# Draghoyns/FLAIR-1

Hardware: AMD Instinct MI355X
Metric: 512x512x5 tiles/s (train fwd+bwd) (higher is better)
Workload: dtype bf16; 1 GPU; U-Net/ResNet34 5-ch 512x512 13-class train step (fwd + fused CE/argmax/confmat + bwd + SGD), bs=32/GPU, random-init weights; global_batch=32, parallelism=dp1, grad_allreduce=none

## Files before the change

flair-1_amd/build.py:

```python
#!/usr/bin/env python3
import os
import subprocess
import sys
from concurrent.futures import ThreadPoolExecutor

HERE = os.path.dirname(os.path.abspath(__file__))
CSRC = os.path.join(HERE, "csrc")
OUT_DIR = os.path.join(HERE, "flair_amd")
OBJ_DIR = os.path.join(HERE, "build")
LIB = os.path.join(OUT_DIR, "libflair_hip.so")
SOURCES = ["conv_igemm.hip", "conv_halo.hip", "conv_hg.hip", "wgrad.hip", "wgrad_halo.hip", "wgrad_hg.hip", "stem.hip", "batchnorm.hip", "misc.hip", "ce_head.hip", "feed.hip", "zone_stitch.hip", "zone_metrics.hip", "tiff_lzw.hip", "tiff_read.hip", "unet.hip", "capi.hip", "prof.hip", "tune.hip", "metadata_mlp.hip", "tf_exec.hip", "segformer_ops.hip", "segformer.hip", "swin_ops.hip", "upernet.hip"]
FLAGS = ["--offload-arch=gfx950", "-O3", "-std=c++17", "-fPIC", "-Wall", "-Wno-unused-function"]
SOURCE_FLAGS = {src: ["-fno-slp-vectorize"] for src in ("feed.hip", "zone_stitch.hip", "zone_metrics.hip")}
if os.environ.get("FLAIR_STAMPS") == "1":
    FLAGS.append("-DFLAIR_HG_STAMPS")


def _hipcc():
    for c in (os.environ.get("HIPCC"), "/opt/rocm/bin/hipcc", "hipcc"):
        if c and (os.path.isabs(c) and os.path.exists(c) or not os.path.isabs(c)):
            return c
    return "hipcc"


def _newer(target, deps):
    if not os.path.exists(target):
        return False
    t = os.path.getmtime(target)
    return all(os.path.getmtime(d) <= t for d in deps)


def build(force=False, verbose=True):
    os.makedirs(OBJ_DIR, exist_ok=True)
    headers = [os.path.join(CSRC, f) for f in os.listdir(CSRC) if f.endswith(".h")]
    headers.append(os.path.join(os.path.dirname(HERE), "include", "flair_hip.h"))
    hipcc = _hipcc()
    jobs = []
    objs = []
    for src in SOURCES:
        s = os.path.join(CSRC, src)
        o = os.path.join(OBJ_DIR, src.replace(".hip", ".o"))
        objs.append(o)
        if force or not _newer(o, [s] + headers):
            jobs.append([hipcc] + FLAGS + SOURCE_FLAGS.get(src, []) + ["-c", s, "-o", o])

    def run(cmd):
        if verbose:
            print(" ".join(cmd), flush=True)
        r = subprocess.run(cmd, capture_output=True, text=True)
        if r.returncode != 0:
            raise RuntimeError("hipcc failed:\n" + " ".join(cmd) + "\n" + r.stdout + r.stderr)
        if verbose and r.stderr.strip():
            print(r.stderr, flush=True)

    with ThreadPoolExecutor(max_workers=4) as ex:
        list(ex.map(run, jobs))
    if force or jobs or not os.path.exists(LIB):
        run([hipcc, "--offload-arch=gfx950", "-shared", "-fPIC", "-o", LIB] + objs)
    return LIB


if __name__ == "__main__":
    print(build(force="--force" in sys.argv))
```

flair-1_amd/csrc/capi.hip:

```cpp
#include <new>
#include <string.h>

#include "../../include/flair_hip.h"
#include "unet.h"
#include "conv_args.h"
#include "parity_pack.h"
#include "segformer.h"
#include "upernet.h"
#include "segformer_ops.h"
#include "swin_ops.h"

using namespace flair;

struct flair_unet { UNet net; flair_unet(int a, int b, int c) : net(a, b, c) {} };
struct flair_segformer {
  SegFormer net;
  flair_segformer(int a, int b, const int* d, const int* h, const int* hd, const int* sr, int dh, int dt) : net(a, b, d, h, hd, sr, dh, dt) {}
};

struct flair_upernet {
  UperNet net;
  flair_upernet(int a, int b, int e, const int* d, const int* h, int hid, const int* ps, int ai, int ac, int dt)
      : net(a, b, e, d, h, hid, ps, ai, ac, dt) {}
};
// ... 468 lines not shown
  ConvArgs a;
  float standin;
  if (!p || conv_ex_fill(p, a)) return 0;
  conv_ex_sizing(p, a, &standin);
  if (p->mode == 2) {
    PackTable tb;
    return conv_ex_parity_packs(p, a, nullptr, tb) + 256;
  }
  a.stats = p->stats;
  size_t b = (size_t)round_up((long)((size_t)conv_weight_rows_pad(p->Cout) * a.Kpad * dtype_size(p->dtype)), 256);
  if (p->stats) b += (size_t)round_up((long)conv_grid_rows(p->dtype, a) * 2 * p->Cout * 4, 256);
  return b + 256;
}

int flair_conv2d_ex_grid_rows(const flair_conv_ex_t* p) {
  ConvArgs a;
  float standin;
  if (!p) return -1;
  const int rc = conv_ex_fill(p, a);
  if (rc) return rc;
  conv_ex_sizing(p, a, &standin);
  a.stats = p->stats;
  return conv_grid_rows(p->dtype, a);
}

int flair_conv2d_ex(const flair_conv_ex_t* p, void* workspace, size_t wsb, void* stream) {
  if (!p || !p->x0 || !p->w_oihw || !workspace) return -1;
  hipStream_t s = (hipStream_t)stream;
  ConvArgs a;
  int rc = conv_ex_fill(p, a);
  if (rc) return rc;
  if (p->mode == 2) {
    if (!p->y_nhwc) return -1;
    PackTable tb;
    if (conv_ex_parity_packs(p, a, (unsigned char*)workspace, tb) > wsb) return -100;
    rc = pack_weights_all(p->dtype, p->w_oihw, workspace, tb, s);
    return rc ? rc : launch_conv(p->dtype, a, s);
  }
  if (p->bnr_partial ? (!p->bnr_y || !p->bnr_scale || !p->bnr_shift) : (p->bnr_y != nullptr)) return -1;
  OpArena ar(workspace, wsb);
  const int Cin = a.C0 + a.C1, rows_f = conv_weight_rows_pad(p->Cout);
  void* wp = ar.get((size_t)rows_f * a.Kpad * dtype_size(p->dtype));
  a.w = wp;
  if (p->bnr_partial && p->bnr_rows < conv_grid_rows(p->dtype, a)) return -100;
  float* partial = nullptr;
  int nblk = 0;
  if (p->stats) {
    a.stats = p->stats;
    nblk = conv_grid_rows(p->dtype, a);
    partial = (float*)ar.get((size_t)nblk * 2 * p->Cout * 4);
    a.stats = partial;
  }
  if (ar.bad) return -100;
  rc = p->mode == 1 ? pack_weight(p->dtype, p->w_oihw, wp, Cin, p->Cout, p->R, p->R, Cin, rows_f, a.Kpad, 1, s)
                    : pack_weight(p->dtype, p->w_oihw, wp, p->Cout, Cin, p->R, p->R, Cin, rows_f, a.Kpad, 0, s);
  if (rc) return rc;
  rc = launch_conv(p->dtype, a, s);
  if (rc) return rc;
  if (p->stats) rc = partial_rows_sum(partial, nblk, 2 * p->Cout, p->stats, s);
  return rc;
}

static int wgrad_ex_fill(const flair_wgrad_ex_t* p, WgradArgs& w) {
  if (p->dtype != DT_F32 && p->dtype != DT_BF16) return -2;
  const ConvInput in{p->x0, p->x1, p->C0, p->x1 ? p->C1 : 0, p->up0, p->N, p->H, p->W};
  wgrad_args(w, in, p->R, p->stride, p->pad, p->dy, p->dy_ld > 0 ? p->dy_ld : p->Cout, p->Cout, p->dw,
             p->Cin_real > 0 ? p->Cin_real : in.C0 + in.C1);
  w.accumulate = p->accumulate; w.in_scale = p->in_scale; w.in_shift = p->in_shift; w.cus = p->cus; w.dbias = p->dbias;
  w.fuse_y = p->fuse_y; w.fuse_coef = p->fuse_coef; w.fuse_msc = p->fuse_msc; w.fuse_msh = p->fuse_msh;
  return 0;
}

size_t flair_conv2d_wgrad_ex_workspace_bytes(const flair_wgrad_ex_t* p) {
  WgradArgs w;
  if (!p || wgrad_ex_fill(p, w)) return 0;
  size_t b = (size_t)round_up((long)wgrad_workspace_bytes(p->dtype, w), 256);
  if (p->dbias && wgrad_dbias_fusable(p->dtype, w)) b += (size_t)round_up((long)WGRAD_DBIAS_ROWS * w.dy_ld * 4, 256);
  return b + 256;
}

int flair_conv2d_wgrad_ex(const flair_wgrad_ex_t* p, void* workspace, size_t wsb, void* stream) {
  if (!p || !p->x0 || !p->dy || !p->dw || !workspace) return -1;
  WgradArgs w;
  int rc = wgrad_ex_fill(p, w);
  if (rc) return rc;
  OpArena ar(workspace, wsb);
  w.partial = (float*)ar.get(wgrad_workspace_bytes(p->dtype, w));
  if (p->dbias && wgrad_dbias_fusable(p->dtype, w)) w.dbias_partial = (float*)ar.get((size_t)WGRAD_DBIAS_ROWS * w.dy_ld * 4);
  if (ar.bad) return -100;
  return launch_wgrad(p->dtype, w, (hipStream_t)stream);
}

size_t flair_bn_workspace_bytes(int64_t rows, int C) {
  if (rows < 1 || C < 1) return 0;
  const size_t partial = (size_t)round_up((long)bn_bwd_blocks(rows) * 2 * C * 4, 256);
  const size_t fwd = 2 * (size_t)round_up((long)C * 4, 256) + partial + (size_t)round_up(2L * C * 4, 256);
  const size_t bwd = partial + (size_t)round_up(3L * C * 4, 256);
  return (fwd > bwd ? fwd : bwd) + 256;
}

int flair_bn_relu_forward(int dtype, const void* y, int64_t rows, int C, const float* gamma, const float* beta,
                          float* running_mean, float* running_var, int training, const void* residual, int relu,
                          void* out, float* save_mean, float* save_invstd, void* workspace, size_t wsb, void* stream) {
  if (!y || !out || !workspace) return -1;
  hipStream_t s = (hipStream_t)stream;
  OpArena ar(workspace, wsb);
  float* scale = (float*)ar.get(C * 4);
  float* shift = (float*)ar.get(C * 4);
  int rc;
  if (training) {
    const int nblk = bn_bwd_blocks(rows);
    float* partial = (float*)ar.get((size_t)nblk * 2 * C * 4);
    float* zo = (float*)ar.get(2 * C * 4);
    if (ar.bad) return -100;
    rc = bn_stats_partial(dtype, y, rows, C, partial, zo, s);
    if (rc) return rc;
    rc = bn_finalize(partial, nblk, C, rows, gamma, beta, running_mean, running_var, 0.1f, 1e-5f, scale, shift,
                     save_mean, save_invstd, s);
  } else {
    if (ar.bad) return -100;
    rc = bn_eval_coeffs(C, gamma, beta, running_mean, running_var, 1e-5f, scale, shift, s);
  }
  if (rc) return rc;
  return bn_act(dtype, y, scale, shift, residual, nullptr, nullptr, out, rows, C, relu, s);
}

int flair_bn_relu_backward(int dtype, const void* dout, const void* out, const void* y, int64_t rows, int C,
                           const float* gamma, const float* save_mean, const float* save_invstd, int relu, void* dy,
                           void* dres, float* dgamma, float* dbeta, void* workspace, size_t wsb, void* stream) {
  if (!dout || !y || !dy || !workspace) return -1;
  OpArena ar(workspace, wsb);
  float* partial = (float*)ar.get((size_t)bn_bwd_blocks(rows) * 2 * C * 4);
  float* coef = (float*)ar.get(3 * C * 4);
  if (ar.bad) return -100;
  return bn_backward(dtype, dout, relu ? out : nullptr, y, save_mean, save_invstd, gamma, rows, C, partial, coef, dgamma,
                     dbeta, 0, dy, dres, 0, nullptr, nullptr, 0, 0, (hipStream_t)stream);
}

int flair_bn_backward_ex(const flair_bn_bwd_ex_t* p, void* workspace, size_t wsb, void* stream) {
  if (!p || !p->dout || !p->y || !p->mean || !p->invstd || !workspace || p->rows < 1 || p->C < 1) return -1;
  if (p->dtype != DT_F32 && p->dtype != DT_BF16) return -2;
  if (p->dres && !p->dy) return -1;
  if (!p->dgamma != !p->dbeta) return -1;
  if (p->pre_nblk > 0 && !p->partial) return -1;
  OpArena ar(workspace, wsb);
  float* partial = p->pre_nblk > 0 ? p->partial : (float*)ar.get((size_t)bn_bwd_blocks(p->rows) * 2 * p->C * 4);
  float* coef = p->coef ? p->coef : (float*)ar.get(3 * (size_t)p->C * 4);
  if (ar.bad) return -100;
  return bn_backward(p->dtype, p->dout, p->out, p->y, p->mean, p->invstd, p->gamma, (long)p->rows, p->C, partial, coef, p->dgamma,
                     p->dbeta, p->accumulate_param, p->dy, p->dres, p->dres_accumulate, p->mscale, p->mshift, p->pre_nblk,
                     p->premasked, (hipStream_t)stream);
}

int flair_maxpool_backward_ex(int dtype, const void* dy, const uint8_t* idx, void* dx, int accumulate, int N, int H, int W, int C,
                              const void* bnr_y, const float* bnr_msc, const float* bnr_msh, float* bnr_partial, void* stream) {
  if (!dy || !idx || !dx || N < 1 || H < 1 || W < 1 || C < 1) return -1;
  if (dtype != DT_F32 && dtype != DT_BF16) return -2;
  return maxpool3x3s2_bwd(dtype, dy, idx, dx, accumulate, N, H, W, C, (hipStream_t)stream, bnr_y, bnr_msc, bnr_msh, bnr_partial);
}
int flair_bn_act(int dtype, const void* y, const float* scale, const float* shift, void* out, int64_t rows, int C, int relu, void* stream) {
  if (!y || !scale || !shift || !out || rows < 1 || C < 1) return -1;
  if (dtype != DT_F32 && dtype != DT_BF16) return -2;
  return bn_act(dtype, y, scale, shift, nullptr, nullptr, nullptr, out, (long)rows, C, relu, (hipStream_t)stream);
}
int flair_bn_act_maxpool(int dtype, const void* y, const float* scale, const float* shift, void* act, void* out, uint8_t* idx, int N,
                         int H, int W, int C, void* stream) {
  if (!y || !scale || !shift || !act || !out || N < 1 || H < 1 || W < 1 || C < 1) return -1;
  if (dtype != DT_F32 && dtype != DT_BF16) return -2;
  return bn_act_maxpool3x3s2(dtype, y, scale, shift, act, out, idx, N, H, W, C, (hipStream_t)stream);
}
int flair_upcat_bwd(int dtype, const void* dcat, void* dx0, int dx0_accumulate, void* dskip, int dskip_accumulate, int N, int H, int W,
                    int C0, int C1, void* stream) {
  if (!dcat || !dx0 || (C1 > 0 && !dskip) || N < 1 || H < 1 || W < 1 || C0 < 1 || C1 < 0) return -1;
  if (dtype != DT_F32 && dtype != DT_BF16) return -2;
  return upcat_bwd(dtype, dcat, dx0, dx0_accumulate, dskip, dskip_accumulate, N, H, W, C0, C1, (hipStream_t)stream);
}
int flair_ew_add(int dtype, void* dst, const void* src, int64_t n, void* stream) {
  if (!dst || !src || n < 1) return -1;
  if (dtype != DT_F32 && dtype != DT_BF16) return -2;
  return ew_add(dtype, dst, src, (long)n, (hipStream_t)stream);
}
int flair_colsum(int dtype, const void* x, int64_t rows, int ld, int C, float* out, void* workspace, size_t wsb, void* stream) {
  if (!x || !out || !workspace || rows < 1 || ld < 1 || C < 1) return -1;
  if (dtype != DT_F32 && dtype != DT_BF16) return -2;
  OpArena ar(workspace, wsb);
  float* partial = (float*)ar.get((size_t)bn_bwd_blocks((long)rows) * ld * 4);
  if (ar.bad) return -100;
  return colsum(dtype, x, (long)rows, ld, C, partial, out, (hipStream_t)stream);
}
int flair_pack_weights(int dtype, const float* params, const flair_pack_desc_t* descs, int n, void* base, void* stream) {
  if (!params || !descs || !base) return -1;
  if ((dtype != DT_F32 && dtype != DT_BF16) || n < 1 || n > PackTable::MAX) return -2;
  PackTable tb;
  tb.n = n;
  for (int i = 0; i < n; ++i) {
    const flair_pack_desc_t& q = descs[i];
    const int taps = q.Rc > 0 ? q.Rc * q.Sc : q.R * q.S;
    if (q.Cout < 1 || q.Cin < 1 || q.R < 1 || q.S < 1 || taps < 1 || (long)taps * q.Cin_p > q.Kpad || q.Cin_p < (q.tf ? q.Cout : q.Cin) ||
        q.rows_pad < (q.tf ? q.Cin : q.Cout) || q.w_off < 0)
      return -2;
    const bool vec = dtype == DT_BF16 && q.R * q.S == 9 &&
                     (q.tf ? ((q.Cin & 31) == 0 && (q.Cout & 31) == 0) : (q.Rc == 0 && (q.Cin & 3) == 0));
    if (vec && (((uintptr_t)params & 15) || (q.w_off & 3))) return -2;
    if (q.Rc > 0 && (q.r0 + (q.Rc - 1) * q.rstep >= q.R || q.s0 + (q.Sc - 1) * q.sstep >= q.S || q.r0 < 0 || q.s0 < 0 || q.rstep < 1 || q.sstep < 1))
      return -2;
    PackDesc& d = tb.d[i];
    memset(&d, 0, sizeof(d));
    d.w_off = (long)q.w_off; d.dst_off = (size_t)q.dst_off; d.Cout = q.Cout; d.Cin = q.Cin; d.R = q.R; d.S = q.S;
    d.Cin_p = q.Cin_p; d.rows_pad = q.rows_pad; d.Kpad = q.Kpad; d.tf = q.tf;
    d.r0 = (unsigned char)q.r0; d.rstep = (unsigned char)q.rstep; d.Rc = (unsigned char)q.Rc;
    d.s0 = (unsigned char)q.s0; d.sstep = (unsigned char)q.sstep; d.Sc = (unsigned char)q.Sc;
  }
  return pack_weights_all(dtype, params, base, tb, (hipStream_t)stream);
}
int flair_pack_weight(int dtype, const float* w_oihw, void* dst, int Cout, int Cin, int R, int S, int Cin_p, int rows_pad, int Kpad,
                      int tf, void* stream) {
  if (!w_oihw || !dst) return -1;
  if (dtype != DT_F32 && dtype != DT_BF16) return -2;
  if (Cout < 1 || Cin < 1 || R < 1 || S < 1 || (long)R * S * Cin_p > Kpad || Cin_p < (tf ? Cout : Cin) || rows_pad < (tf ? Cin : Cout))
    return -2;
  return pack_weight(dtype, w_oihw, dst, Cout, Cin, R, S, Cin_p, rows_pad, Kpad, tf ? 1 : 0, (hipStream_t)stream);
}

int flair_maxpool_forward(int dtype, const void* x, void* y, uint8_t* idx, int N, int H, int W, int C, void* stream) {
  return maxpool3x3s2_fwd(dtype, x, y, idx, N, H, W, C, (hipStream_t)stream);
}
int flair_maxpool_backward(int dtype, const void* dy, const uint8_t* idx, void* dx, int N, int H, int W, int C, void* stream) {
  return maxpool3x3s2_bwd(dtype, dy, idx, dx, 0, N, H, W, C, (hipStream_t)stream);
}
int flair_nchw_to_nhwc(int dtype, const float* x, void* y, int N, int C, int H, int W, int Cpad, void* stream) {
  return nchw_f32_to_nhwc(dtype, x, y, N, C, H, W, Cpad, (hipStream_t)stream);
}
int flair_nhwc_to_nchw(int dtype, const void* x, float* y, int N, int C, int H, int W, int Cpad, void* stream) {
  return nhwc_to_nchw_f32(dtype, x, y, N, C, H, W, Cpad, nullptr, (hipStream_t)stream);
}

#define FLAIR_DT_OK(dt) ((dt) == DT_F32 || (dt) == DT_BF16)
int flair_sf_layernorm(int dtype, const void* x, const float* gamma, const float* beta, void* y, int64_t rows, int C, float eps, void* stream) {
  if (!x || !gamma || !beta || !y || rows < 1 || C < 1) return -1;
  if (!FLAIR_DT_OK(dtype)) return -2;
  return sf_layernorm(dtype, x, gamma, beta, y, (long)rows, C, eps, (hipStream_t)stream);
}
int flair_sf_dwconv3x3_gelu(int dtype, const void* x, const float* w, const float* bias, void* y, int B, int H, int W, int C, void* stream) {
  if (!x || !w || !bias || !y || B < 1 || H < 1 || W < 1 || C < 1) return -1;
  if (!FLAIR_DT_OK(dtype)) return -2;
  return sf_dwconv3x3_gelu(dtype, x, w, bias, y, B, H, W, C, (hipStream_t)stream);
}
int flair_sf_bilinear_nhwc(int dtype, const void* x, void* y, int B, int h, int w, int C, int H, int W, int ld, void* stream) {
  if (!x || !y || B < 1 || h < 1 || w < 1 || H < 1 || W < 1 || C < 1 || ld < C) return -1;
  if (!FLAIR_DT_OK(dtype)) return -2;
  return sf_bilinear_nhwc(dtype, x, y, B, h, w, C, H, W, ld, (hipStream_t)stream);
}
int flair_sf_bilinear_nchw_f32(const float* x, float* y, int64_t planes, int h, int w, int H, int W, void* stream) {
  if (!x || !y || planes < 1 || h < 1 || w < 1 || H < 1 || W < 1) return -1;
  return sf_bilinear_nchw_f32(x, y, (long)planes, h, w, H, W, (hipStream_t)stream);
}
int flair_sf_slice_cols(int dtype, const float* src, int ld, int col0, int ncols, int64_t rows, void* dst, void* stream) {
  if (!src || !dst || rows < 1 || col0 < 0 || ncols < 1 || col0 + ncols > ld) return -1;
  if (!FLAIR_DT_OK(dtype)) return -2;
  return sf_slice_cols(dtype, src, ld, col0, ncols, (long)rows, dst, (hipStream_t)stream);
}
int flair_sf_fuse_bias(const float* wf, int D, const float* b3, const float* b2, const float* b1, const float* b0, const float* scale,
                       const float* shift, float* shift2, void* stream) {
  if (!wf || !b3 || !b2 || !b1 || !b0 || !scale || !shift || !shift2 || D < 1) return -1;
  return sf_fuse_bias(wf, D, b3, b2, b1, b0, scale, shift, shift2, (hipStream_t)stream);
}
int flair_sf_upsample_sum_bn_relu(int dtype, const void* g0, const void* g1, const void* g2, const void* g3, const float* scale,
                                  const float* shift2, void* z, int B, int H, int W, int D, void* stream) {
  if (!g0 || !g1 || !g2 || !g3 || !scale || !shift2 || !z || B < 1 || H < 1 || W < 1 || D < 1) return -1;
  if (!FLAIR_DT_OK(dtype)) return -2;
  return sf_upsample_sum_bn_relu(dtype, g0, g1, g2, g3, scale, shift2, z, B, H, W, D, (hipStream_t)stream);
}
int flair_sf_ffn_fused_ok(int dtype, int C, int H, int W) { return sf_ffn_fused_ok(dtype, C, H, W) ? 1 : 0; }
int flair_sf_ffn_dw_pack(const float* w, const float* b, float* out, int nch, void* stream) {
  if (!w || !b || !out || nch < 1) return -1;
  return sf_ffn_dw_pack(w, b, out, nch, (hipStream_t)stream);
}
int flair_sf_ffn_fused(const void* x, const float* ln_g, const float* ln_b, const void* w1, const float* b1, const float* dwp, const void* w2,
                       const float* b2, void* out, int B, int H, int W, int C, float eps, const float* ln2_g, const float* ln2_b, void* out_ln,
                       void* stream) {
  if (!x || !ln_g || !ln_b || !w1 || !b1 || !dwp || !w2 || !b2 || !out || B < 1) return -1;
  return sf_ffn_fused(x, ln_g, ln_b, w1, b1, dwp, w2, b2, out, B, H, W, C, eps, ln2_g, ln2_b, out_ln, (hipStream_t)stream);
}
int flair_sf_head_fused_ok(int dtype, int H, int W, int C0, int D, int labels) { return sf_head_fused_ok(dtype, H, W, C0, D, labels) ? 1 : 0; }
int flair_sf_head_wint(void* wint, void* stream) {
  if (!wint) return -1;
  return sf_head_wint(wint, (hipStream_t)stream);
}
int flair_sf_head_fused(const void* f0, const void* w0, const void* g1, const void* g2, const void* g3, const void* wint, const float* scale,
                        const float* shift2, const void* wc, const float* bc, float* out, int B, int H, int W, int D, int labels, void* stream) {
  if (!f0 || !w0 || !g1 || !g2 || !g3 || !wint || !scale || !shift2 || !wc || !out || B < 1 || labels < 1) return -1;
  return sf_head_fused(f0, w0, g1, g2, g3, wint, scale, shift2, wc, bc, out, B, H, W, D, labels, (hipStream_t)stream);
}
int flair_sf_attention(int dtype, const void* q, const void* k, const void* v, void* out, int B, int N, int Nk, int hidden, int kv_ld,
                       void* stream) {
  if (!q || !k || !v || !out || B < 1 || N < 1 || hidden < 1) return -1;
  if (!FLAIR_DT_OK(dtype)) return -2;
  return sf_attention(dtype, q, k, v, out, B, N, Nk, hidden, kv_ld, (hipStream_t)stream);
}
int flair_swin_window_attention(int dtype, const void* qkv, const float* qkv_bias, const float* table, void* out, int B, int H, int W, int C,
                                int heads, int shift, void* stream) {
  if (!qkv || !qkv_bias || !table || !out) return -1;
  if (!FLAIR_DT_OK(dtype)) return -2;
  return swin_window_attention(dtype, qkv, qkv_bias, table, out, B, H, W, C, heads, shift, (hipStream_t)stream);
}
int flair_swin_layernorm(int dtype, const void* x, const float* gamma, const float* beta, void* y, int64_t rows, int C, int ld, float eps,
// ... 144 lines not shown
```

flair-1_amd/csrc/unet.h:

```cpp
#pragma once
#include <string>
#include <vector>

#include "ops.h"

namespace flair {

struct Act {
  void* p = nullptr;
  int N = 0, H = 0, W = 0, C = 0;
  const float* lz_scale = nullptr;
  const float* lz_shift = nullptr;
  long rows() const { return (long)N * H * W; }
  long elems() const { return rows() * C; }
};

struct ConvDesc {
  std::string name;
  int Cin, Cout, R, S, stride, pad;
  int Cin_p, Cout_p;
  bool bias;
  long w_off = -1, b_off = -1;
  size_t wf = 0, wd = 0;
  int Kpad, rows_f;
  int Kpad_d, rows_d;
  size_t wd_cls[4] = {0, 0, 0, 0};
  int Kpad_cls[4] = {0, 0, 0, 0};
  bool parity_dgrad() const { return stride == 2 && R == 3 && S == 3 && pad == 1; }
};

struct BnDesc {
  std::string name;
  int C;
  long g_off, b_off;
  long rm_off, rv_off;
};

struct TensorInfo {
  std::string name;
  int ndim;
  long shape[4];
  long offset;
  int kind;
  int stage;
};

struct Unit {
  int conv = -1, bn = -1;
  Act in0, in1;
  bool up0 = false;
  Act y, out;
  float *scale = nullptr, *shift = nullptr, *mean = nullptr, *invstd = nullptr;
  bool relu = true;
  int res_unit = -1;
  Act res;
  float* bnr_partial = nullptr;
  int bnr_nblk = 0;
  bool bnr_masked = false;
};

struct FwdOpts {
  bool reuse_constants = false;
  unsigned char* preds = nullptr;
  float* maxprob = nullptr;
  struct Ce {
    const void* labels = nullptr; int kind = 0; const float* weight = nullptr;
    float* loss = nullptr; unsigned char* preds = nullptr; long long* confmat = nullptr; float* ws = nullptr;
  } ce;
  const float* rows = nullptr;
  float* drows = nullptr;
  int refusal(int training, bool fp32_logits, int H, int W) const;
};

class UNet {
 public:
  UNet(int in_channels, int classes, int dtype);
  int in_channels, classes, dtype;
  std::vector<ConvDesc> convs;
  std::vector<BnDesc> bns;
  std::vector<TensorInfo> tensors;
  long n_params = 0, n_buffers = 0;
  long stage_begin[8];

  size_t workspace_bytes(int B, int H, int W, int training) const;

  int forward(const float* params, float* buffers, const float* x_nchw, float* logits_nchw, int B, int H, int W,
              int training, void* ws, size_t ws_bytes, hipStream_t s, const FwdOpts& o);
  int backward(const float* params, const float* dlogits_nchw, const void* dlogits_nhwc, float* grads, void* ws,
               size_t ws_bytes, hipStream_t s, void* const* stage_events = nullptr);

  int encoder_forward(const float* params, float* buffers, const float* x_nchw, float* const feats_nchw[5], int B,
                      int H, int W, int training, void* ws, size_t ws_bytes, hipStream_t s);
  int decoder_forward(const float* params, float* buffers, const float* const feats_nchw[5], float* out_nchw, int B,
                      int H, int W, int training, void* ws, size_t ws_bytes, hipStream_t s);
  int head_forward(const float* params, const float* x_nchw, float* logits_nchw, int B, int H, int W, int training,
                   void* ws, size_t ws_bytes, hipStream_t s);
  int head_backward(const float* params, const float* dlogits_nchw, float* dx_nchw, float* grads, void* ws,
                    size_t ws_bytes, hipStream_t s);
  int decoder_backward(const float* params, const float* dout_nchw, float* const dfeats_nchw[5], float* grads,
                       void* ws, size_t ws_bytes, hipStream_t s);
  int encoder_backward(const float* params, const float* const dfeats_nchw[5], float* grads, void* ws,
                       size_t ws_bytes, hipStream_t s);

  void invalidate_reuse() { last_valid_ = false; last_params_ = nullptr; last_buffers_ = nullptr; }
  void* last_dlogits_nhwc() const { return dl_nhwc_; }
  const void* logits_nhwc() const { return logits_nhwc_; }
  int head_ld() const { return convs.back().Cout_p; }

 private:
  unsigned char* base_ = nullptr;
  size_t cap_ = 0, top_ = 0;
  bool dry_ = false;
  int err_ = 0;
  hipStream_t s_ = nullptr;
  void* alloc(size_t bytes);
  Act alloc_act(int N, int H, int W, int C);
  float* alloc_f(long n) { return (float*)alloc((size_t)n * 4); }

  const float* params_ = nullptr;
  float* buffers_ = nullptr;
  float* grads_ = nullptr;
  int B_ = 0, H_ = 0, W_ = 0, training_ = 0;
  std::vector<Unit> units_;
  Act xin_, f_[6], dec_in_[6], pool_, dec_out_;
  unsigned char* pool_idx_ = nullptr;
  int enc_units_end_ = 0, dec_units_begin_ = 0;
  size_t fwd_top_ = 0;
  bool packed_d_ = false;
  bool reuse_ = false, last_valid_ = false;
  const void* last_ws_ = nullptr;
  const void* last_params_ = nullptr;
  const void* last_buffers_ = nullptr;
  int last_B_ = 0, last_H_ = 0, last_W_ = 0;
  bool lazy_ok_ = false;
  int lazy_max_c_ = 16;
  hipStream_t side_ = nullptr;
  hipStream_t note_ = nullptr;
  std::vector<hipEvent_t> fork_ev_;
  hipEvent_t join_ev_ = nullptr;
  size_t fork_next_ = 0;
  bool side_pending_ = false;
  Act f5m_;
  float* drows_pending_ = nullptr;
  bool side_init();
  hipStream_t wgrad_stream();
  int side_cus() const;
  void side_join();
 public:
  ~UNet();
 private:
  void* dl_nhwc_ = nullptr;
  void* logits_nhwc_ = nullptr;
  void* const* stage_events_ = nullptr;
  void stage_done(int stage);

  struct GradBuf { void* act; void* g; bool init; };
  int sole_producer(const Act& a) const;
  int residual_producer(const Act& a) const;
  void attach_bn_reduce(ConvArgs& a, const Act& target);
  std::vector<GradBuf> gbufs_;
  const void* acc_src_next_ = nullptr;
  bool bwd_fuse() const;
  void* grad_of(const Act& a, bool* accumulate);
  void* grad_peek(const Act& a);

  size_t plan_bytes(int B, int H, int W, int training);
  void build_table();
  int add_conv(const std::string& name, int cin, int cout, int k, int stride, int pad, bool bias, int stage);
  int add_bn(const std::string& name, int c, int stage);
  void begin(void* ws, size_t ws_bytes, hipStream_t s, bool dry);
  void pack_forward_weights();
  void pack_dgrad_weights();
  int run_unit(int conv, int bn, const Act& in0, const Act& in1, bool up0, bool relu, int res_unit, const Act& res,
               bool materialize, int lazy_cons = -1, bool lazy_up0 = false, const Act* lazy_skip = nullptr);
  bool lazy_into_hg(const Act& y, int cons, bool up0, const Act& skip) const;
  void encoder_fwd_impl(const float* x_nchw);
  void decoder_fwd_impl();
  void head_fwd_impl(float* logits_nchw, const FwdOpts& o);
  void unit_backward(int ui, const void* dout, void* dres, bool dres_acc, bool need_dgrad, void* dx_override,
                     bool upcat = false);
  void head_bwd_impl(const void* dl);
  void decoder_bwd_impl();
  void encoder_bwd_impl();
  void fwd_common_begin(const float* params, float* buffers, int B, int H, int W, int training);
};

}
```

flair-1_amd/csrc/unet.hip:

```cpp
#include <stdlib.h>

#include "unet.h"
#include "conv_args.h"
#include "conv_route.h"
#include "parity_pack.h"
#include "tune.h"

namespace flair {

#define RUN(expr)                         \
  do {                                    \
    if (!dry_ && !err_) {                 \
      int rc__ = (expr);                  \
      if (rc__) err_ = rc__;              \
    }                                     \
  } while (0)

int UNet::add_conv(const std::string& name, int cin, int cout, int k, int stride, int pad, bool bias, int stage) {
  ConvDesc c;
  c.name = name; c.Cin = cin; c.Cout = cout; c.R = k; c.S = k; c.stride = stride; c.pad = pad; c.bias = bias;
  c.Cin_p = (int)round_up(cin, 8);
  c.Cout_p = (int)round_up(cout < 16 ? 16 : cout, 16);
  c.w_off = n_params;
  TensorInfo t;
// ... 392 lines not shown

int FwdOpts::refusal(int training, bool fp32_logits, int H, int W) const {
  if ((maxprob && !preds) || (drows && !rows)) return -1;
  if (ce.labels && (!ce.loss || !ce.ws || ce.kind < 0 || ce.kind > 3)) return -1;
  if (ce.labels && (preds || training || fp32_logits)) return -15;
  if (rows && training && !drows) return -16;
  if (drows && !training) return -17;
  if ((H % 32) || (W % 32)) return -10;
  return 0;
}

int UNet::forward(const float* params, float* buffers, const float* x_nchw, float* logits_nchw, int B, int H, int W,
                  int training, void* ws, size_t ws_bytes, hipStream_t s, const FwdOpts& o) {
  if (const int rc = o.refusal(training, logits_nchw != nullptr, H, W)) return rc;
  f5m_ = Act(); drows_pending_ = nullptr;
  reuse_ = o.reuse_constants && !training && last_valid_ && ws == last_ws_ && params == last_params_ && buffers == last_buffers_ &&
           B == last_B_ && H == last_H_ && W == last_W_;
  begin(ws, ws_bytes, s, false);
  fwd_common_begin(params, buffers, B, H, W, training);
  const int lazy_env = tune("FLAIR_LAZY_BN", 1);
  lazy_ok_ = lazy_env != 0;
  lazy_max_c_ = lazy_env >= 2 ? 32 : 16;
  if (!reuse_) pack_forward_weights();
  encoder_fwd_impl(x_nchw);
  if (o.rows && !training) RUN(add_rowvec_nhwc(dtype, f_[5].p, o.rows, f_[5].N, f_[5].H, f_[5].W, f_[5].C, s_));
  const Act f5 = f_[5];
  if (o.rows && training) {
    f5m_ = alloc_act(f5.N, f5.H, f5.W, f5.C);
    RUN(add_rowvec_nhwc_to(dtype, f5.p, o.rows, f5m_.p, f5.N, f5.H, f5.W, f5.C, s_));
    f_[5] = f5m_;
    drows_pending_ = o.drows;
  }
  decoder_fwd_impl();
  f_[5] = f5;
  head_fwd_impl(logits_nchw, o);
  fwd_top_ = top_;
  reuse_ = false;
  last_valid_ = !training && !err_;
  last_ws_ = ws; last_params_ = params; last_buffers_ = buffers; last_B_ = B; last_H_ = H; last_W_ = W;
  return err_;
}

int UNet::encoder_forward(const float* params, float* buffers, const float* x_nchw, float* const feats[5], int B, int H,
                          int W, int training, void* ws, size_t ws_bytes, hipStream_t s) {
  invalidate_reuse();
  f5m_ = Act(); drows_pending_ = nullptr;
  if ((H % 32) || (W % 32)) return -10;
  begin(ws, ws_bytes, s, false);
  fwd_common_begin(params, buffers, B, H, W, training);
  lazy_ok_ = false;
  pack_forward_weights();
  encoder_fwd_impl(x_nchw);
  for (int i = 0; i < 5; ++i) {
    const Act& f = f_[i + 1];
    RUN(nhwc_to_nchw_f32(dtype, f.p, feats[i], f.N, f.C, f.H, f.W, f.C, nullptr, s_));
  }
  fwd_top_ = top_;
  return err_;
}

int UNet::decoder_forward(const float* params, float* buffers, const float* const feats[5], float* out_nchw, int B, int H,
                          int W, int training, void* ws, size_t ws_bytes, hipStream_t s) {
  invalidate_reuse();
  if (ws != base_ || B != B_ || H != H_ || W != W_) return -11;
  s_ = s; training_ = training; params_ = params; buffers_ = buffers;
  for (int i = 0; i < 5; ++i) {
    Act f = alloc_act(f_[i + 1].N, f_[i + 1].H, f_[i + 1].W, f_[i + 1].C);
    RUN(nchw_f32_to_nhwc(dtype, feats[i], f.p, f.N, f.C, f.H, f.W, f.C, s_));
    dec_in_[i + 1] = f;
  }
  Act saved[6];
  for (int i = 1; i <= 5; ++i) { saved[i] = f_[i]; f_[i] = dec_in_[i]; }
  decoder_fwd_impl();
  for (int i = 1; i <= 5; ++i) f_[i] = saved[i];
  RUN(nhwc_to_nchw_f32(dtype, dec_out_.p, out_nchw, dec_out_.N, 16, dec_out_.H, dec_out_.W, dec_out_.C, nullptr, s_));
  fwd_top_ = top_;
  return err_;
}

int UNet::head_forward(const float* params, const float* x_nchw, float* logits_nchw, int B, int H, int W, int training,
                       void* ws, size_t ws_bytes, hipStream_t s) {
  invalidate_reuse();
  if (ws != base_ || B != B_ || H != H_ || W != W_) return -11;
  s_ = s; params_ = params; training_ = training;
  Act x = alloc_act(B, H, W, 16);
  RUN(nchw_f32_to_nhwc(dtype, x_nchw, x.p, B, 16, H, W, 16, s_));
  dec_out_ = x;
  head_fwd_impl(logits_nchw, FwdOpts());
  fwd_top_ = top_;
  return err_;
}

int UNet::sole_producer(const Act& a) const {
  if (!a.p) return -1;
  for (int i = 0; i < (int)units_.size(); ++i) {
    const Unit& u = units_[i];
    if (u.out.p != a.p) continue;
    const bool mask_from_y = u.relu && u.res_unit < 0 && !u.res.p;
    if (!mask_from_y) return -1;
    int consumers = 0;
    for (const Unit& v : units_) consumers += (v.in0.p == a.p) + (v.in1.p == a.p) + (v.res.p == a.p);
    for (int f = 1; f <= 5; ++f) consumers += (f_[f].p == a.p);
    if (a.p == dec_out_.p) consumers += 1;
    return consumers == 1 ? i : -1;
  }
  return -1;
}

int UNet::residual_producer(const Act& a) const {
  if (!a.p) return -1;
  for (int f = 1; f <= 5; ++f)
    if (f_[f].p == a.p) return -1;
  if (a.p == dec_out_.p) return -1;
  for (int i = 0; i < (int)units_.size(); ++i) {
    const Unit& u = units_[i];
    if (u.out.p != a.p) continue;
    if (!u.relu || (u.res_unit < 0 && !u.res.p)) return -1;
    int convs_in = 0, res_in = 0;
    for (const Unit& v : units_) { convs_in += (v.in0.p == a.p) + (v.in1.p == a.p); res_in += (v.res.p == a.p); }
    return (convs_in == 1 && res_in == 1) ? i : -1;
  }
  return -1;
}

void UNet::attach_bn_reduce(ConvArgs& a, const Act& target) {
  const int mode = tune("FLAIR_BNR_RES", 1);
  int p = sole_producer(target);
  bool from_out = false;
  if (p < 0 && a.accumulate && mode) { p = residual_producer(target); from_out = p >= 0; }
  if (p < 0) return;
  Unit& u = units_[p];
  a.bnr_y = u.y.p; a.bnr_scale = u.scale; a.bnr_shift = u.shift; a.bnr_C = u.y.C;
  a.bnr_out = from_out ? u.out.p : nullptr;
  a.bnr_partial = reinterpret_cast<float*>(1);
  if ((a.accumulate && !from_out) || u.y.C != a.out_ld || !conv_tile_epilogue_ok(dtype, a) || !conv_mfma_bound(dtype, a)) {
    a.bnr_y = nullptr; a.bnr_out = nullptr; a.bnr_partial = nullptr; a.bnr_scale = a.bnr_shift = nullptr; a.bnr_C = 0;
    return;
  }
  const int nblk = conv_grid_rows(dtype, a);
  a.bnr_partial = alloc_f((long)nblk * 2 * u.y.C);
  u.bnr_partial = a.bnr_partial;
  u.bnr_nblk = nblk;
  if (bwd_fuse() && conv_family(dtype, a) == CONV_HG) { a.bnr_mask = 1; u.bnr_masked = true; }
}

bool UNet::bwd_fuse() const { return tune("FLAIR_BWD_FUSE", 1) != 0; }

void UNet::unit_backward(int ui, const void* dout, void* dres, bool dres_acc, bool need_dgrad, void* dx_override,
                         bool upcat) {
  Unit& u = units_[ui];
  const ConvDesc& c = convs[u.conv];
  const BnDesc& b = bns[u.bn];
  const long rows = u.y.rows();
  void* dy = alloc((size_t)u.y.elems() * dtype_size(dtype));
  const int pre_nblk = u.bnr_nblk;
  const bool masked = u.bnr_masked && pre_nblk > 0;
  float* partial = pre_nblk > 0 ? u.bnr_partial : alloc_f((long)bn_bwd_blocks(rows) * 2 * b.C);
  u.bnr_partial = nullptr; u.bnr_nblk = 0; u.bnr_masked = false;
  float* coef = alloc_f(3 * b.C);
  const void* acc_src = acc_src_next_;
  acc_src_next_ = nullptr;
  const bool mask_from_y = u.relu && u.res_unit < 0 && !u.res.p;
  WgradArgs w;
  wgrad_args(w, conv_input(u.in0, u.in1, u.up0), c.R, c.stride, c.pad, dy, u.y.C, c.Cout, grads_ + c.w_off, c.Cin);
  const bool fuse_apply = !need_dgrad && !dres && mask_from_y && wgrad_bnapply_fusable(dtype, w);

  enum { DG_NONE, DG_PLAIN, DG_UPCAT_TILE, DG_UPCAT_SPLIT, DG_PARITY } dg = DG_NONE;
  ConvArgs a;
  void *dx0 = nullptr, *dsk = nullptr, *dcat = nullptr;
  bool acc0 = false, acc1 = false;
  if (need_dgrad) {
    dg = DG_PLAIN;
    conv_dgrad_args(a, dtype, ConvInput{dy, nullptr, u.y.C, 0, 0, u.y.N, u.y.H, u.y.W}, c.R, c.stride, c.pad, w.Hin, w.Win, c.Cin_p);
    a.w = base_ + c.wd;
    a.out_ld = c.Cin_p;
    if (upcat) {
      const int C0 = u.in0.C, C1 = u.in1.p ? u.in1.C : 0;
      dx0 = grad_of(u.in0, &acc0);
      dsk = C1 ? grad_of(u.in1, &acc1) : nullptr;
      a.pool_c0 = C0; a.out = dx0; a.out_ld = C0; a.accumulate = acc0 ? 1 : 0;
      a.out_skip = dsk; a.out_skip_ld = C1; a.skip_accumulate = acc1 ? 1 : 0;
      if (conv_tile_epilogue_ok(dtype, a)) {
        dg = DG_UPCAT_TILE;
        attach_bn_reduce(a, u.in0);
        if (drows_pending_ && u.in0.p == f5m_.p && (a.bnr_partial || a.bnr_mask) && !err_) err_ = -18;
      } else {
        dg = DG_UPCAT_SPLIT;
        dcat = alloc((size_t)u.y.rows() * (C0 + C1) * dtype_size(dtype));
        a.pool_c0 = 0; a.out_skip = nullptr; a.out = dcat; a.out_ld = C0 + C1; a.accumulate = 0;
      }
    } else {
      if (dx_override) {
        a.out = dx_override; a.accumulate = 0;
      } else {
        bool acc = false;
        a.out = grad_of(u.in0, &acc);
        a.accumulate = acc ? 1 : 0;
        if (acc_src) {
          ConvArgs t = a;
          t.accumulate = 1; t.acc_src = acc_src;
          if (!acc && conv_acc_src_ok(dtype, t)) {
            a = t;
          } else {
            if (acc) RUN(ew_add(dtype, a.out, acc_src, u.in0.elems(), s_));
            else if (!dry_ && !err_ && hipMemcpyAsync(a.out, acc_src, (size_t)u.in0.elems() * dtype_size(dtype), hipMemcpyDeviceToDevice, s_) != hipSuccess) err_ = -14;
            a.accumulate = 1;
          }
        }
        attach_bn_reduce(a, u.in0);
      }
      const bool doubled = c.stride == 2 && a.Hout == 2 * u.y.H && a.Wout == 2 * u.y.W;
      if (doubled && (c.parity_dgrad() || (c.R == 1 && c.S == 1 && c.pad == 0 && a.accumulate))) {
        dg = DG_PARITY;
        conv_parity_args(a, dtype, c.R);
        if (a.ncls) {
          a.w = base_ + c.wd_cls[3];
          for (int cls = 0; cls < 4; ++cls) a.cls_w[cls] = base_ + c.wd_cls[cls];
        }
      }
    }
  }
  const bool nomask = masked && !dres && bwd_fuse();
  RUN(bn_backward(dtype, dout, (u.relu && !mask_from_y && !nomask) ? u.out.p : nullptr, u.y.p, u.mean, u.invstd, params_ + b.g_off,
                  rows, b.C, partial, coef, grads_ + b.g_off, grads_ + b.b_off, 0, fuse_apply ? nullptr : dy, dres,
                  dres_acc ? 1 : 0, (mask_from_y && !nomask) ? u.scale : nullptr, (mask_from_y && !nomask) ? u.shift : nullptr,
                  pre_nblk, nomask ? 1 : 0, s_));
  if (fuse_apply) { w.dy = dout; w.fuse_y = u.y.p; w.fuse_coef = coef; w.fuse_msc = u.scale; w.fuse_msh = u.shift; }
  w.in_scale = u.in0.lz_scale; w.in_shift = u.in0.lz_shift;
  w.cus = side_cus();
  w.partial = (float*)alloc(wgrad_workspace_bytes(dtype, w));
  {
    hipStream_t ws = wgrad_stream();
    RUN(launch_wgrad(dtype, w, ws));
  }
  switch (dg) {
    case DG_NONE: break;
    case DG_UPCAT_SPLIT:
      RUN(launch_conv(dtype, a, s_));
      RUN(upcat_bwd(dtype, dcat, dx0, acc0 ? 1 : 0, dsk, acc1 ? 1 : 0, u.y.N, u.y.H, u.y.W, u.in0.C, u.in1.p ? u.in1.C : 0, s_));
      break;
    default:
      RUN(launch_conv(dtype, a, s_));
  }
}

void UNet::head_bwd_impl(const void* dl) {
  const ConvDesc& c = convs.back();
  Act none;
  WgradArgs w;
  wgrad_args(w, conv_input(dec_out_, none, false), c.R, c.stride, c.pad, dl, c.Cout_p, c.Cout, grads_ + c.w_off, c.Cin);
  w.in_scale = dec_out_.lz_scale; w.in_shift = dec_out_.lz_shift;
  w.partial = (float*)alloc(wgrad_workspace_bytes(dtype, w));
  const bool fuse_db = wgrad_dbias_fusable(dtype, w);
  if (fuse_db) { w.dbias = grads_ + c.b_off; w.dbias_partial = alloc_f((long)WGRAD_DBIAS_ROWS * c.Cout_p); }
  {
    hipStream_t ws = wgrad_stream();
    RUN(launch_wgrad(dtype, w, ws));
  }
  if (!fuse_db) {
    const long rows = dec_out_.rows();
    float* partial = alloc_f((long)bn_bwd_blocks(rows) * c.Cout_p);
    RUN(colsum(dtype, dl, rows, c.Cout_p, c.Cout, partial, grads_ + c.b_off, s_));
  }
  ConvArgs a;
  conv_dgrad_args(a, dtype, ConvInput{dl, nullptr, c.Cout_p, 0, 0, dec_out_.N, dec_out_.H, dec_out_.W}, c.R, c.stride, c.pad, dec_out_.H,
                  dec_out_.W, c.Cin_p);
  a.w = base_ + c.wd;
  bool acc = false;
  a.out = grad_of(dec_out_, &acc);
  a.out_ld = c.Cin_p; a.accumulate = acc ? 1 : 0;
  attach_bn_reduce(a, dec_out_);
  RUN(launch_conv(dtype, a, s_));
}

void UNet::decoder_bwd_impl() {
  for (int i = 4; i >= 0; --i) {
    const int u1 = dec_units_begin_ + 2 * i, u2 = u1 + 1;
    unit_backward(u2, grad_peek(units_[u2].out), nullptr, false, true, nullptr);
    unit_backward(u1, grad_peek(units_[u1].out), nullptr, false, true, nullptr, true);
  }
}

void UNet::encoder_bwd_impl() {
  int ui = enc_units_end_ - 1;
  const int nblk[4] = {3, 4, 6, 3};
  for (int L = 3; L >= 0; --L) {
    for (int b = nblk[L] - 1; b >= 0; --b) {
      const bool ds = (b == 0 && L > 0);
      const int u2 = ui, ud = ds ? ui - 1 : -1, u1 = ds ? ui - 2 : ui - 1;
      ui = u1 - 1;
      const Act& X = units_[u1].in0;
      const void* dO = grad_peek(units_[u2].out);
      const bool dz_ready = units_[u2].bnr_masked && units_[u2].bnr_nblk > 0 && bwd_fuse();
      if (!ds) {
        if (dz_ready) {
          unit_backward(u2, dO, nullptr, false, true, nullptr);
          acc_src_next_ = dO;
        } else {
          bool acc = false;
          void* dX = grad_of(X, &acc);
          unit_backward(u2, dO, dX, acc, true, nullptr);
        }
      } else {
        void* dz = dz_ready ? const_cast<void*>(dO) : alloc((size_t)units_[u2].y.elems() * dtype_size(dtype));
        unit_backward(u2, dO, dz_ready ? nullptr : dz, false, true, nullptr);
        unit_backward(u1, grad_peek(units_[u1].out), nullptr, false, true, nullptr);
        unit_backward(ud, dz, nullptr, false, true, nullptr);
        continue;
      }
      unit_backward(u1, grad_peek(units_[u1].out), nullptr, false, true, nullptr);
    }
    stage_done(L + 1);
  }
  bool acc = false;
  void* df1 = grad_of(f_[1], &acc);
  {
    Unit& u0 = units_[0];
    const bool fuse = tune("FLAIR_POOL_BNR", 1) && u0.relu && u0.res_unit < 0 && !u0.res.p && u0.y.C == 64;
    float* part = nullptr;
    const int nblk = B_ * f_[1].H;
    if (fuse) { part = alloc_f((long)nblk * 2 * u0.y.C); u0.bnr_partial = part; u0.bnr_nblk = nblk; }
    RUN(maxpool3x3s2_bwd(dtype, grad_peek(pool_), pool_idx_, df1, acc ? 1 : 0, B_, f_[1].H, f_[1].W, 64, s_,
                         fuse ? u0.y.p : nullptr, fuse ? u0.scale : nullptr, fuse ? u0.shift : nullptr, part));
  }
  unit_backward(0, df1, nullptr, false, false, nullptr);
  stage_done(0);
}

void UNet::stage_done(int stage) {
  const bool listened = stage_events_ && stage_events_[stage] && !dry_ && !err_;
  if (stage == 0) side_join();
  if (!listened) return;
  hipEvent_t ev = (hipEvent_t)stage_events_[stage];
  if (stage != 0 && side_pending_) {
    if (!note_) {
      int least = 0, greatest = 0;
      const int np = tune("FLAIR_NOTE_PRIO", 1);
      hipError_t ce;
      if (np && hipDeviceGetStreamPriorityRange(&least, &greatest) == hipSuccess && least != greatest)
        ce = hipStreamCreateWithPriority(&note_, hipStreamNonBlocking, np == 2 ? greatest : least);
      else
        ce = hipStreamCreateWithFlags(&note_, hipStreamNonBlocking);
      if (ce != hipSuccess) note_ = nullptr;
    }
    if (note_) {
      hipEvent_t e1 = fork_ev_[fork_next_++ % fork_ev_.size()];
      hipEvent_t e2 = fork_ev_[fork_next_++ % fork_ev_.size()];
      hipError_t e = hipEventRecord(e1, s_);
      if (e == hipSuccess) e = hipEventRecord(e2, side_);
      if (e == hipSuccess) e = hipStreamWaitEvent(note_, e1, 0);
      if (e == hipSuccess) e = hipStreamWaitEvent(note_, e2, 0);
      if (e == hipSuccess) e = hipEventRecord(ev, note_);
      if (e != hipSuccess) err_ = (int)e;
      return;
    }
    side_join();
  }
  const hipError_t e = hipEventRecord(ev, s_);
  if (e != hipSuccess) err_ = (int)e;
}

int UNet::backward(const float* params, const float* dlogits_nchw, const void* dlogits_nhwc, float* grads, void* ws,
                   size_t ws_bytes, hipStream_t s, void* const* stage_events) {
  invalidate_reuse();
  if (ws != base_ || !training_) return -11;
  s_ = s; params_ = params; grads_ = grads; top_ = fwd_top_;
  stage_events_ = stage_events;
  gbufs_.clear();
  pack_dgrad_weights();
  const void* dl = dlogits_nhwc;
  if (!dl) {
    const int ld = convs.back().Cout_p;
    void* t = alloc((size_t)dec_out_.rows() * ld * dtype_size(dtype));
    RUN(nchw_f32_to_nhwc(dtype, dlogits_nchw, t, B_, classes, H_, W_, ld, s_));
    dl = t;
  }
  head_bwd_impl(dl);
  stage_done(6);
  decoder_bwd_impl();
  stage_done(5);
  if (drows_pending_) {
    float* const drows = drows_pending_;
    drows_pending_ = nullptr;
    void* g = grad_peek(f5m_);
    if (!g) { if (!err_) err_ = -11; }
    else {
      RUN(rowvec_grad_nhwc(dtype, g, drows, f5m_.N, f5m_.H, f5m_.W, f5m_.C, s_));
      for (auto& gb : gbufs_)
        if (gb.act == f5m_.p) gb.act = f_[5].p;
    }
  }
  encoder_bwd_impl();
  stage_events_ = nullptr;
  return err_;
}

int UNet::head_backward(const float* params, const float* dlogits_nchw, float* dx_nchw, float* grads, void* ws,
                        size_t ws_bytes, hipStream_t s) {
  invalidate_reuse();
  if (ws != base_ || !training_) return -11;
  s_ = s; params_ = params; grads_ = grads;
  pack_dgrad_weights();
  const int ld = convs.back().Cout_p;
  void* t = alloc((size_t)dec_out_.rows() * ld * dtype_size(dtype));
  RUN(nchw_f32_to_nhwc(dtype, dlogits_nchw, t, B_, classes, H_, W_, ld, s_));
  head_bwd_impl(t);
  side_join();
  RUN(nhwc_to_nchw_f32(dtype, grad_peek(dec_out_), dx_nchw, B_, 16, H_, W_, 16, nullptr, s_));
  return err_;
}

int UNet::decoder_backward(const float* params, const float* dout_nchw, float* const dfeats[5], float* grads, void* ws,
                           size_t ws_bytes, hipStream_t s) {
  invalidate_reuse();
  if (ws != base_ || !training_) return -11;
  s_ = s; params_ = params; grads_ = grads;
  pack_dgrad_weights();
  const Act& out = units_.back().out;
  bool acc = false;
  void* g = grad_of(out, &acc);
  RUN(nchw_f32_to_nhwc(dtype, dout_nchw, g, out.N, 16, out.H, out.W, out.C, s_));
  decoder_bwd_impl();
  side_join();
  for (int i = 0; i < 5; ++i) {
    const Act& f = dec_in_[i + 1];
    RUN(nhwc_to_nchw_f32(dtype, grad_peek(f), dfeats[i], f.N, f.C, f.H, f.W, f.C, nullptr, s_));
  }
  return err_;
}

int UNet::encoder_backward(const float* params, const float* const dfeats[5], float* grads, void* ws, size_t ws_bytes,
                           hipStream_t s) {
  invalidate_reuse();
  if (ws != base_ || !training_) return -11;
  s_ = s; params_ = params; grads_ = grads;
  pack_dgrad_weights();
  for (int i = 0; i < 5; ++i) {
    const Act& f = f_[i + 1];
    bool acc = false;
    void* g = grad_of(f, &acc);
    if (acc) { if (!err_) err_ = -12; }
    RUN(nchw_f32_to_nhwc(dtype, dfeats[i], g, f.N, f.C, f.H, f.W, f.C, s_));
  }
  encoder_bwd_impl();
  return err_;
}

size_t UNet::workspace_bytes(int B, int H, int W, int training) const {
  UNet scratch(in_channels, classes, dtype);
  return scratch.plan_bytes(B, H, W, training);
}

size_t UNet::plan_bytes(int B, int H, int W, int training) {
  begin(nullptr, 0, nullptr, true);
  fwd_common_begin(nullptr, nullptr, B, H, W, training);
  lazy_ok_ = false;
  encoder_fwd_impl(nullptr);
  Act saved[6];
  for (int i = 1; i <= 5; ++i) {
    dec_in_[i] = alloc_act(f_[i].N, f_[i].H, f_[i].W, f_[i].C);
    saved[i] = f_[i];
    f_[i] = dec_in_[i];
  }
  decoder_fwd_impl();
  for (int i = 1; i <= 5; ++i) f_[i] = saved[i];
  dec_out_ = alloc_act(B, H, W, 16);
  head_fwd_impl(nullptr, FwdOpts());
  if (training) {
    alloc((size_t)dec_out_.rows() * convs.back().Cout_p * dtype_size(dtype));
    grads_ = nullptr;
    head_bwd_impl(nullptr);
    bool acc;
    grad_of(units_.back().out, &acc);
    decoder_bwd_impl();
    for (int i = 1; i <= 5; ++i) grad_of(f_[i], &acc);
    encoder_bwd_impl();
  }
  const size_t need = top_ + (1 << 20);
  dry_ = false;
  base_ = nullptr;
  units_.clear();
  gbufs_.clear();
  return need;
}

}
```

flair-1_amd/csrc/wgrad_halo.hip:

```cpp
#include "common.h"
#include "halo_stage.h"
#include "launch.h"
#include "mma.h"
#include "tune.h"
#include "ops.h"

namespace flair {

void launch_wgrad_reduce(const float* partial, float* dw, int splits, int Cout, int Cout_pad, int Kpad, int Cin,
                         int Cin_real, int R, int S, int accumulate, hipStream_t s);

namespace {

constexpr int TH = 8, TW = 32, HH = TH + 2, HW_ = TW + 2, HPIX = HH * HW_;

template <typename T> struct HFrag;
template <> struct HFrag<bf16_t> {
  static constexpr int KSTEP = 32;
  template <int STRIDE>
  __device__ static __forceinline__ u32x4 load(const unsigned char* img, int row0, int cb, int lane) {
    const int g = lane >> 4, i = lane & 15, q = i >> 2, p = i & 3;
    typedef __attribute__((address_space(3))) s16x4_t* lds_p;
    s16x4_t lo = __builtin_amdgcn_ds_read_tr16_b64_v4i16((lds_p)(img + (row0 + 8 * g + 2 * q) * STRIDE + cb + 8 * p));
    s16x4_t hi = __builtin_amdgcn_ds_read_tr16_b64_v4i16((lds_p)(img + (row0 + 8 * g + 2 * q + 1) * STRIDE + cb + 8 * p));
    u32x4 r;
    r.x = (unsigned)(unsigned short)lo[0] | ((unsigned)(unsigned short)lo[1] << 16);
    r.y = (unsigned)(unsigned short)lo[2] | ((unsigned)(unsigned short)lo[3] << 16);
    r.z = (unsigned)(unsigned short)hi[0] | ((unsigned)(unsigned short)hi[1] << 16);
    r.w = (unsigned)(unsigned short)hi[2] | ((unsigned)(unsigned short)hi[3] << 16);
    return r;
  }
};
template <> struct HFrag<float> {
  static constexpr int KSTEP = 16;
  template <int STRIDE>
  __device__ static __forceinline__ u32x4 load(const unsigned char* img, int row0, int cb, int lane) {
    const int g = lane >> 4, i = lane & 15;
    u32x4 r;
    r.x = *reinterpret_cast<const unsigned*>(img + (row0 + g) * STRIDE + cb + 4 * i);
    r.y = *reinterpret_cast<const unsigned*>(img + (row0 + 4 + g) * STRIDE + cb + 4 * i);
    r.z = *reinterpret_cast<const unsigned*>(img + (row0 + 8 + g) * STRIDE + cb + 4 * i);
    r.w = *reinterpret_cast<const unsigned*>(img + (row0 + 12 + g) * STRIDE + cb + 4 * i);
    return r;
  }
};

struct WgHaloArgs {
  const void* x0; const void* x1; int C0, C1, up0;
  int N, H, W;
  const void* dy; int dy_ld; int Cout;
  float* partial;
  int Cout_pad, Kg;
  int ntiles;
  const float* in_scale; const float* in_shift;
  float* dbias_partial;
};

template <typename T, int CK, int CO>
struct WgHaloCfg {
  static constexpr int CH = Elem<T>::CH;
  static constexpr int CPP = CK / CH;
  static constexpr int DPP = CO / CH;
  static constexpr int XSTRIDE = CK * (int)sizeof(T) + 16;
  static constexpr int DSTRIDE = CO * (int)sizeof(T) + 16;
  static constexpr int XBYTES = HPIX * XSTRIDE;
  static constexpr int DBYTES = TH * TW * DSTRIDE;
  static constexpr int COT = CO / 16, CIT = CK / 16, NT = COT * CIT * 9;
  static constexpr int RED = NT * 4 * 64 * 4;
  static constexpr int STAGE = XBYTES + DBYTES;
  static constexpr int SMEM = STAGE > RED ? STAGE : RED;
  static constexpr int XITEMS = (HPIX * CPP + 255) / 256;
  static constexpr int DITEMS = (TH * TW * DPP + 255) / 256;
};

template <typename T, int CK, int CO, bool LZ, bool DB = false>
__global__ __launch_bounds__(256) void wgrad3x3_halo_kernel(const WgHaloArgs a) {
  using Cfg = WgHaloCfg<T, CK, CO>;
  constexpr int CH = Cfg::CH, CPP = Cfg::CPP, DPP = Cfg::DPP, COT = Cfg::COT, CIT = Cfg::CIT;
  constexpr int KSTEP = HFrag<T>::KSTEP;
  extern __shared__ __attribute__((aligned(16))) unsigned char smem[];
  unsigned char* xh = smem;
  unsigned char* dyt = smem + Cfg::XBYTES;
  const int t = threadIdx.x, lane = t & 63, wave = t >> 6;
  const int H = a.H, W = a.W;
  const int tiles_x = W / TW, tiles_y = H / TH;
  const int cbase = blockIdx.y * CK;
  const int kbase = blockIdx.z * CO;
  const T* __restrict__ x0 = (const T*)a.x0;
  const T* __restrict__ x1 = (const T*)a.x1;
  const T* __restrict__ dy = (const T*)a.dy;
  const bool use0 = cbase < a.C0;
  const T* __restrict__ xb = use0 ? x0 : x1;
  const int Hs = (use0 && a.up0) ? (H >> 1) : H, Ws = (use0 && a.up0) ? (W >> 1) : W, Cs = use0 ? a.C0 : a.C1;
  const int sh = (use0 && a.up0) ? 1 : 0;
  const int coff = use0 ? cbase : cbase - a.C0;

  constexpr int WC = COT * CIT, WK = 4 / WC, ROWS = TH / WK;
  static_assert(WC == 1 || WC == 2 || WC == 4, "wave mapping");
  const int combo = wave % WC, kp = wave / WC;
  const int co = combo / CIT, ci = combo % CIT;
  f32x4_t acc[9];
#pragma unroll
  for (int tp = 0; tp < 9; ++tp) acc[tp] = f32x4_t{0.f, 0.f, 0.f, 0.f};
  float lsc[CH], lsh[CH];
  if (LZ && a.in_scale) lazy_coef_load<T, CPP>(a.in_scale, a.in_shift, cbase, t, lsc, lsh);

  u32x4 xrA[Cfg::XITEMS], drA[Cfg::DITEMS], xrB[Cfg::XITEMS], drB[Cfg::DITEMS];
  unsigned xbitsA = 0, dbitsA = 0, xbitsB = 0, dbitsB = 0;
  auto load_tile = [&](int tile, u32x4 (&xr)[Cfg::XITEMS], u32x4 (&dr)[Cfg::DITEMS], unsigned& xbits, unsigned& dbits) {
    const bool tok = tile < a.ntiles;
    int n, y0, x0p;
    tile_decode<TW, TH>(tok ? tile : 0, tiles_x, tiles_y, n, y0, x0p);
    unsigned xb2 = 0, db2 = 0;
#pragma unroll
    for (int k = 0; k < Cfg::XITEMS; ++k) {
      const int it = t + 256 * k;
      const int hp = it / CPP, ch = it - hp * CPP;
      const int hy = hp / HW_, hx = hp - hy * HW_;
      const int iy = y0 - 1 + hy, ix = x0p - 1 + hx;
      const bool ok = tok && (it < HPIX * CPP) && ((unsigned)iy < (unsigned)H) && ((unsigned)ix < (unsigned)W);
      const unsigned off = ok ? (unsigned)(((n * Hs + (iy >> sh)) * Ws + (ix >> sh)) * Cs + coff + ch * CH) : 0u;
      xr[k] = *reinterpret_cast<const u32x4*>(xb + off);
      xb2 |= (ok ? 1u : 0u) << k;
    }
#pragma unroll
    for (int k = 0; k < Cfg::DITEMS; ++k) {
      const int it = t + 256 * k;
      const int px = it / DPP, ch = it - px * DPP;
      const int py = px / TW, pxx = px - py * TW;
      const int col = kbase + ch * CH;
      const bool ok = tok && (it < TH * TW * DPP) && col < a.dy_ld;
      const unsigned off = ok ? (unsigned)(((n * H + y0 + py) * W + x0p + pxx) * a.dy_ld + col) : 0u;
      dr[k] = *reinterpret_cast<const u32x4*>(dy + off);
      db2 |= (ok ? 1u : 0u) << k;
    }
    xbits = xb2; dbits = db2;
  };
  load_tile(blockIdx.x, xrA, drA, xbitsA, dbitsA);
  load_tile(blockIdx.x + gridDim.x, xrB, drB, xbitsB, dbitsB);
  float bsum[CH];
  if constexpr (DB) {
    static_assert(256 % DPP == 0, "a thread keeps one dY chunk column");
#pragma unroll
    for (int e = 0; e < CH; ++e) bsum[e] = 0.f;
  }
  auto do_tile = [&](int tile, u32x4 (&xr)[Cfg::XITEMS], u32x4 (&dr)[Cfg::DITEMS], unsigned& xbits, unsigned& dbits) {
    __syncthreads();
    halo_put<T, TW, TH, CPP, 256, Cfg::XITEMS, HaloRows<Cfg::XSTRIDE>, LZ>(xh, t, xr, xbits, a.in_scale != nullptr, lsc, lsh);
#pragma unroll
    for (int k = 0; k < Cfg::DITEMS; ++k) {
      const int it = t + 256 * k;
      if (it < TH * TW * DPP) {
        const int px = it / DPP, ch = it - px * DPP;
        const u32x4 dv = dr[k] & (0u - ((dbits >> k) & 1u));
        *reinterpret_cast<u32x4*>(dyt + px * Cfg::DSTRIDE + ch * 16) = dv;
        if constexpr (DB) {
          float f[CH];
          chunk_to_f<T>(__builtin_bit_cast(uint4, dv), f);
#pragma unroll
          for (int e = 0; e < CH; ++e) bsum[e] += f[e];
        }
      }
    }
    load_tile(tile + 2 * gridDim.x, xr, dr, xbits, dbits);
    __builtin_amdgcn_sched_barrier(0);
    __syncthreads();
#pragma unroll
    for (int yy = 0; yy < ROWS; ++yy) {
      const int y = kp * ROWS + yy;
#pragma unroll
      for (int xs = 0; xs < TW; xs += KSTEP) {
        const u32x4 af = HFrag<T>::template load<Cfg::DSTRIDE>(dyt, y * TW + xs, co * 16 * (int)sizeof(T), lane);
#pragma unroll
        for (int tp = 0; tp < 9; ++tp) {
          const int r = tp / 3, s = tp - 3 * r;
          const u32x4 bf = HFrag<T>::template load<Cfg::XSTRIDE>(xh, (y + r) * HW_ + xs + s, ci * 16 * (int)sizeof(T), lane);
          Mma<T>::run(af, bf, acc[tp]);
        }
      }
    }
  };
  for (int tile = blockIdx.x; tile < a.ntiles; tile += 2 * gridDim.x) {
    do_tile(tile, xrA, drA, xbitsA, dbitsA);
    if (tile + gridDim.x < a.ntiles) do_tile(tile + gridDim.x, xrB, drB, xbitsB, dbitsB);
  }

  if constexpr (DB) {
    __syncthreads();
    float* bs = reinterpret_cast<float*>(smem);
#pragma unroll
    for (int e = 0; e < CH; ++e) bs[t * CH + e] = bsum[e];
    __syncthreads();
    if (t < CO) {
      const int chunk = t / CH, e = t - chunk * CH;
      float x = 0.f;
      for (int th = chunk; th < 256; th += DPP) x += bs[th * CH + e];
      a.dbias_partial[(long)(kbase + t) * gridDim.x + blockIdx.x] = x;
    }
// ... 142 lines not shown
```

flair-1_amd/flair_amd/_lib.py:

```python
from __future__ import annotations

import ctypes as C
import os

import torch

_HERE = os.path.dirname(os.path.abspath(__file__))
LIB_PATH = os.environ.get("FLAIR_HIP_LIB") or os.path.join(_HERE, "libflair_hip.so")

_lib = None

vp, i32, i64, f32, sz = C.c_void_p, C.c_int, C.c_int64, C.c_float, C.c_size_t

PROTOTYPES = {
    "flair_strerror": (C.c_char_p, [i32]),
    "flair_version": (i32, []),
    "flair_unet_create": (i32, [C.POINTER(vp), i32, i32, i32]),
    "flair_unet_destroy": (None, [vp]),
    "flair_unet_param_count": (i64, [vp]),
    "flair_unet_buffer_count": (i64, [vp]),
    "flair_unet_num_tensors": (i32, [vp]),
    "flair_unet_tensor_info": (i32, [vp, i32, C.c_char_p, i32, C.POINTER(i64), C.POINTER(i32), C.POINTER(i64),
                                     C.POINTER(i32), C.POINTER(i32)]),
    "flair_unet_stage_range": (i32, [vp, i32, C.POINTER(i64), C.POINTER(i64)]),
    "flair_unet_workspace_bytes": (i64, [vp, i32, i32, i32, i32]),
    "flair_unet_forward": (i32, [vp, vp, vp, vp, vp, i32, i32, i32, i32, vp, sz, vp, vp]),
    "flair_unet_backward": (i32, [vp, vp, vp, vp, vp, vp, sz, vp, C.POINTER(vp)]),
    "flair_unet_head_ld": (i32, [vp]),
    "flair_unet_encoder_forward": (i32, [vp, vp, vp, vp, C.POINTER(vp), i32, i32, i32, i32, vp, sz, vp]),
    "flair_unet_decoder_forward": (i32, [vp, vp, vp, C.POINTER(vp), vp, i32, i32, i32, i32, vp, sz, vp]),
    "flair_unet_head_forward": (i32, [vp, vp, vp, vp, i32, i32, i32, i32, vp, sz, vp]),
    "flair_unet_head_backward": (i32, [vp, vp, vp, vp, vp, vp, sz, vp]),
    "flair_unet_decoder_backward": (i32, [vp, vp, vp, C.POINTER(vp), vp, vp, sz, vp]),
    "flair_unet_encoder_backward": (i32, [vp, vp, C.POINTER(vp), vp, vp, sz, vp]),
    "flair_ce_workspace_bytes": (sz, [i32, i32, i32]),
    "flair_ce_head": (i32, [vp, vp, i32, vp, i32, i32, i32, i32, vp, vp, vp, i32, i32, vp, vp, vp, vp, vp, vp]),
    "flair_unet_logits_nhwc": (vp, [vp]),
    "flair_ce_head_nhwc": (i32, [vp, i32, i32, vp, i32, vp, i32, i32, i32, i32, vp, vp, vp, vp, vp, vp, vp]),
    "flair_softmax_argmax_nhwc": (i32, [vp, i32, i32, i32, i32, i32, i32, vp, vp, vp, vp]),
    "flair_softmax_argmax": (i32, [vp, i32, i32, i32, i32, vp, vp, vp, vp]),
    "flair_confmat_update": (i32, [vp, i32, vp, i32, i64, i32, vp, vp]),
    "flair_jaccard": (i32, [vp, i32, vp, vp, vp, vp]),
    "flair_confmat_masks": (i32, [vp, vp, i64, i32, i32, vp, vp]),
    "flair_feed_tiles": (i32, [vp, vp, vp, i32, i32, i32, i32, C.POINTER(i32), i32, i32, C.POINTER(C.c_double),
                               C.POINTER(C.c_double), i32, vp, vp, vp]),
    "flair_feed_tiles_ptrs": (i32, [vp, vp, vp, i32, i32, i32, i32, C.POINTER(i32), i32, i32, C.POINTER(C.c_double),
                                    C.POINTER(C.c_double), i32, vp, vp, vp]),
    "flair_detect_convert": (i32, [vp, i32, i32, i32, i32, i32, vp, vp]),
    "flair_gather_tiles": (i32, [vp, i32, i32, i32, vp, i32, i32, C.POINTER(i32), i32, i32, C.POINTER(C.c_double),
                                 C.POINTER(C.c_double), vp, vp]),
    "flair_detect_stitch": (i32, [vp, i32, i32, i32, i32, i32, vp, vp, i32, i32, vp]),
    "flair_sgd_step": (i32, [vp, vp, i64, f32, vp]),
    "flair_add_rowvec_nchw": (i32, [vp, vp, i32, i32, i32, i32, vp]),
    "flair_add_rowvec_nhwc": (i32, [i32, vp, vp, i32, i32, i32, i32, vp]),
    "flair_add_rowvec_nhwc_to": (i32, [i32, vp, vp, vp, i32, i32, i32, i32, vp]),
    "flair_rowvec_grad_nhwc": (i32, [i32, vp, vp, i32, i32, i32, i32, vp]),
    "flair_conv2d_workspace_bytes": (sz, [i32, i32, i32, i32, i32, i32, i32, i32, i32, i32, i32]),
    "flair_conv2d_forward": (i32, [i32, vp, vp, i32, i32, i32, i32, i32, i32, vp, vp, i32, i32, i32, i32, vp, vp, vp,
                                   vp, sz, vp]),
    "flair_conv2d_backward": (i32, [i32, vp, i32, i32, i32, i32, vp, i32, i32, i32, i32, vp, vp, vp, vp, sz, vp]),
    "flair_conv2d_ex_workspace_bytes": (sz, [vp]),
    "flair_conv2d_ex": (i32, [vp, vp, sz, vp]),
    "flair_conv2d_ex_grid_rows": (i32, [vp]),
    "flair_conv2d_wgrad_ex_workspace_bytes": (sz, [vp]),
    "flair_conv2d_wgrad_ex": (i32, [vp, vp, sz, vp]),
    "flair_bn_workspace_bytes": (sz, [i64, i32]),
    "flair_bn_relu_forward": (i32, [i32, vp, i64, i32, vp, vp, vp, vp, i32, vp, i32, vp, vp, vp, vp, sz, vp]),
    "flair_bn_relu_backward": (i32, [i32, vp, vp, vp, i64, i32, vp, vp, vp, i32, vp, vp, vp, vp, vp, sz, vp]),
    "flair_bn_backward_ex": (i32, [vp, vp, sz, vp]),
    "flair_maxpool_backward_ex": (i32, [i32, vp, vp, vp, i32, i32, i32, i32, i32, vp, vp, vp, vp, vp]),
    "flair_bn_act": (i32, [i32, vp, vp, vp, vp, i64, i32, i32, vp]),
    "flair_bn_act_maxpool": (i32, [i32, vp, vp, vp, vp, vp, vp, i32, i32, i32, i32, vp]),
    "flair_upcat_bwd": (i32, [i32, vp, vp, i32, vp, i32, i32, i32, i32, i32, i32, vp]),
    "flair_ew_add": (i32, [i32, vp, vp, i64, vp]),
    "flair_colsum": (i32, [i32, vp, i64, i32, i32, vp, vp, sz, vp]),
    "flair_pack_weights": (i32, [i32, vp, vp, i32, vp, vp]),
    "flair_pack_weight": (i32, [i32, vp, vp, i32, i32, i32, i32, i32, i32, i32, i32, vp]),
    "flair_maxpool_forward": (i32, [i32, vp, vp, vp, i32, i32, i32, i32, vp]),
    "flair_maxpool_backward": (i32, [i32, vp, vp, vp, i32, i32, i32, i32, vp]),
    "flair_nchw_to_nhwc": (i32, [i32, vp, vp, i32, i32, i32, i32, i32, vp]),
    "flair_nhwc_to_nchw": (i32, [i32, vp, vp, i32, i32, i32, i32, i32, vp]),
    "flair_sf_layernorm": (i32, [i32, vp, vp, vp, vp, i64, i32, f32, vp]),
    "flair_sf_dwconv3x3_gelu": (i32, [i32, vp, vp, vp, vp, i32, i32, i32, i32, vp]),
    "flair_sf_bilinear_nhwc": (i32, [i32, vp, vp, i32, i32, i32, i32, i32, i32, i32, vp]),
    "flair_sf_bilinear_nchw_f32": (i32, [vp, vp, i64, i32, i32, i32, i32, vp]),
    "flair_sf_slice_cols": (i32, [i32, vp, i32, i32, i32, i64, vp, vp]),
    "flair_sf_fuse_bias": (i32, [vp, i32, vp, vp, vp, vp, vp, vp, vp, vp]),
    "flair_sf_upsample_sum_bn_relu": (i32, [i32, vp, vp, vp, vp, vp, vp, vp, i32, i32, i32, i32, vp]),
    "flair_sf_ffn_fused_ok": (i32, [i32, i32, i32, i32]),
    "flair_sf_ffn_dw_pack": (i32, [vp, vp, vp, i32, vp]),
    "flair_sf_ffn_fused": (i32, [vp, vp, vp, vp, vp, vp, vp, vp, vp, i32, i32, i32, i32, f32, vp, vp, vp, vp]),
    "flair_sf_head_fused_ok": (i32, [i32, i32, i32, i32, i32, i32]),
    "flair_sf_head_wint": (i32, [vp, vp]),
    "flair_sf_head_fused": (i32, [vp, vp, vp, vp, vp, vp, vp, vp, vp, vp, vp, i32, i32, i32, i32, i32, vp]),
    "flair_sf_attention": (i32, [i32, vp, vp, vp, vp, i32, i32, i32, i32, i32, vp]),
    "flair_swin_window_attention": (i32, [i32, vp, vp, vp, vp, i32, i32, i32, i32, i32, i32, vp]),
    "flair_swin_layernorm": (i32, [i32, vp, vp, vp, vp, i64, i32, i32, f32, vp]),
    "flair_swin_patch_merge_ln": (i32, [i32, vp, vp, vp, vp, i32, i32, i32, i32, f32, vp]),
    "flair_swin_adaptive_avgpool": (i32, [i32, vp, i32, vp, i32, i32, i32, i32, i32, vp]),
    "flair_swin_bilinear_add": (i32, [i32, vp, vp, i32, i32, i32, i32, i32, i32, vp]),
    "flair_profile_start": (i32, [i32]),
    "flair_profile_stop": (i32, []),
    "flair_profile_kernel": (i32, [i32, C.c_char_p, i32, C.POINTER(C.c_double), C.POINTER(i64), C.POINTER(C.c_double),
                                   C.POINTER(C.c_double)]),
    "flair_metadata_mlp_forward": (i32, [vp, vp, vp, vp, vp, vp, vp, i32, vp]),
    "flair_metadata_mlp_backward": (i32, [vp, vp, vp, vp, vp, vp, vp, i32, vp, vp, vp, vp]),
    "flair_detect_stitch_preds": (i32, [vp, vp, i32, i32, i32, vp, vp, i32, i32, vp]),
    "flair_detect_blend_accum": (i32, [vp, i32, i32, i32, i32, vp, vp, i32, i32, i32, i32, vp, i32, i32, vp]),
    "flair_detect_blend_flush": (i32, [vp, i32, i32, i32, i32, vp, i32, i32, vp]),
    "flair_detect_stitch_max": (i32, [vp, i32, i32, i32, i32, vp, i32, i32, i32, i32, vp, i32, i32, vp]),
    "flair_detect_stitch_max_preds": (i32, [vp, vp, i32, i32, i32, vp, i32, i32, i32, i32, vp, i32, i32, vp]),
    "flair_zone_window_confmat_preds": (i32, [vp, i32, i32, i32, i32, vp, vp, i32, i32, vp, vp]),
    "flair_zone_window_confmat_logits": (i32, [vp, i32, i32, i32, i32, vp, vp, i32, i32, vp, vp]),
    "flair_detect_convert_q4": (i32, [vp, i32, i32, i32, i32, i32, vp, vp]),
    "flair_detect_stitch_q4": (i32, [vp, i32, i32, i32, i32, i32, vp, vp, i32, i32, vp]),
    "flair_detect_blend_accum_q4": (i32, [vp, i32, i32, i32, i32, vp, vp, i32, i32, i32, i32, vp, i32, i32, vp]),
    "flair_detect_stitch_max_q4": (i32, [vp, i32, i32, i32, i32, vp, i32, i32, i32, i32, vp, i32, i32, vp]),
    "flair_zone_window_confmat_logits_q4": (i32, [vp, i32, i32, i32, i32, vp, vp, i32, i32, vp, vp]),
    "flair_zone_window_confmat_raster": (i32, [vp, i32, i32, i32, i32, vp, vp, i32, i32, vp, vp]),
    "flair_zone_raster_confmat": (i32, [vp, vp, i32, i32, i32, vp, vp]),
    "flair_zone_error_map": (i32, [vp, vp, i32, i32, i32, vp, i32, vp, i32, C.c_double, i32, vp, vp, vp, vp, vp, vp]),
    "flair_tiff_lzw_slot_bytes": (C.c_long, [i32, i32]),
    "flair_tiff_lzw_encode": (i32, [vp, i32, i32, i32, i32, vp, C.c_long, vp, vp]),
    "flair_tiff_lzw_tile_slot_bytes": (C.c_long, [i32, i32]),
    "flair_tiff_lzw_encode_tiles": (i32, [vp, i32, vp, i32, i32, i32, i32, i32, C.c_long, C.c_long, vp, C.c_long, vp, vp]),
    "flair_tiff_pack_streams": (i32, [vp, C.c_long, vp, vp, C.c_long, vp, C.c_long, vp]),
    "flair_tiff_lzw_decode_max_strip": (i32, []),
    "flair_tiff_lzw_decode": (i32, [vp, C.c_long, vp, vp, vp, vp, vp, C.c_long, vp, C.c_long, vp, vp]),
    "flair_tiff_lzw_decode_chunks_cap": (i32, []),
    "flair_tiff_lzw_decode_chunks_window": (i32, []),
    "flair_tiff_lzw_decode_chunks": (i32, [vp, C.c_long, vp, vp, vp, vp, C.c_long, vp, C.c_long, vp, vp]),
    "flair_tiff_chunks_to_planes": (i32, [vp, C.c_long, vp, vp, C.c_long, i32, i32, i32, vp, i32, i32, i32, vp]),
    "flair_tiff_chunks_to_batch": (i32, [vp, C.c_long, vp, vp, C.c_long, i32, vp, i32, i32, i32, vp]),
    "flair_segformer_create": (i32, [C.POINTER(vp), i32, i32, C.POINTER(i32), C.POINTER(i32), C.POINTER(i32), C.POINTER(i32), i32, i32]),
    "flair_segformer_destroy": (None, [vp]),
    "flair_segformer_param_count": (i64, [vp]),
    "flair_segformer_num_tensors": (i32, [vp]),
    "flair_segformer_tensor_info": (i32, [vp, i32, C.c_char_p, i32, C.POINTER(i64), C.POINTER(i32), C.POINTER(i64), C.POINTER(i32)]),
    "flair_segformer_workspace_bytes": (i64, [vp, i32, i32, i32]),
    "flair_segformer_weights_changed": (None, [vp]),
    "flair_segformer_forward": (i32, [vp, vp, vp, vp, vp, i32, i32, i32, vp, sz, vp]),
    "flair_upernet_create": (i32, [C.POINTER(vp), i32, i32, i32, C.POINTER(i32), C.POINTER(i32), i32, i32, C.POINTER(i32), i32, i32, i32]),
    "flair_upernet_destroy": (None, [vp]),
    "flair_upernet_param_count": (i64, [vp]),
    "flair_upernet_num_tensors": (i32, [vp]),
    "flair_upernet_tensor_info": (i32, [vp, i32, C.c_char_p, i32, C.POINTER(i64), C.POINTER(i32), C.POINTER(i64), C.POINTER(i32)]),
    "flair_upernet_workspace_bytes": (i64, [vp, i32, i32, i32]),
    "flair_upernet_weights_changed": (None, [vp]),
    "flair_upernet_forward": (i32, [vp, vp, vp, vp, i32, i32, i32, vp, sz, vp]),
    "flair_upernet_forward_quarter": (i32, [vp, vp, vp, vp, i32, i32, i32, vp, sz, vp]),
    "flair_tune_set": (i32, [C.c_char_p, i32]),
    "flair_debug_buffer": (i32, [vp]),
}


class UnetFwdOpts(C.Structure):
    _fields_ = [("reuse_constants", i32), ("preds_u8", vp), ("maxprob_f32", vp),
                ("ce_labels", vp), ("ce_label_kind", i32), ("ce_class_weight", vp), ("ce_loss", vp),
                ("ce_preds_u8", vp), ("ce_confmat", vp), ("ce_workspace", vp),
                ("rows_f32", vp), ("drows_f32", vp)]


class ConvEx(C.Structure):
    _fields_ = [("dtype", i32), ("mode", i32), ("x0", vp), ("x1", vp),
                ("N", i32), ("H", i32), ("W", i32), ("C0", i32), ("C1", i32), ("up0", i32),
                ("w_oihw", vp), ("bias", vp), ("Cout", i32), ("R", i32), ("stride", i32), ("pad", i32),
                ("y_nhwc", vp), ("out_ld", i32), ("y_nchw", vp), ("stats", vp),
                ("in_scale", vp), ("in_shift", vp), ("oscale", vp), ("oshift", vp), ("ores", vp), ("orelu", i32),
                ("accumulate", i32), ("acc_src", vp),
                ("pool_c0", i32), ("out_skip", vp), ("out_skip_ld", i32), ("skip_accumulate", i32),
                ("preds_u8", vp), ("maxprob_f32", vp), ("ogelu", i32),
                ("bnr_y", vp), ("bnr_out", vp), ("bnr_scale", vp), ("bnr_shift", vp),
                ("bnr_partial", vp), ("bnr_rows", i32), ("bnr_mask", i32)]


class WgradEx(C.Structure):
    _fields_ = [("dtype", i32), ("x0", vp), ("x1", vp),
                ("N", i32), ("H", i32), ("W", i32), ("C0", i32), ("C1", i32), ("up0", i32),
                ("dy", vp), ("dy_ld", i32), ("Cout", i32), ("R", i32), ("stride", i32), ("pad", i32),
                ("dw", vp), ("Cin_real", i32), ("accumulate", i32), ("in_scale", vp), ("in_shift", vp),
                ("dbias", vp), ("cus", i32),
                ("fuse_y", vp), ("fuse_coef", vp), ("fuse_msc", vp), ("fuse_msh", vp)]


class BnBwdEx(C.Structure):
    _fields_ = [("dtype", i32), ("dout", vp), ("out", vp), ("y", vp), ("mean", vp), ("invstd", vp), ("gamma", vp),
                ("rows", i64), ("C", i32), ("partial", vp), ("pre_nblk", i32), ("premasked", i32),
                ("mscale", vp), ("mshift", vp), ("dgamma", vp), ("dbeta", vp), ("accumulate_param", i32),
                ("dy", vp), ("dres", vp), ("dres_accumulate", i32), ("coef", vp)]


class PackDesc(C.Structure):
    _fields_ = [("w_off", i64), ("dst_off", C.c_uint64),
                ("Cout", i32), ("Cin", i32), ("R", i32), ("S", i32), ("Cin_p", i32), ("rows_pad", i32), ("Kpad", i32), ("tf", i32),
                ("r0", i32), ("rstep", i32), ("Rc", i32), ("s0", i32), ("sstep", i32), ("Sc", i32)]


class FlairHipError(RuntimeError):
    pass


def lib():
    global _lib
    if _lib is None:
        if not os.path.exists(LIB_PATH):
            raise FlairHipError(
                f"{LIB_PATH} not found: the HIP extension is required (no CPU fallback). "
                "Build it with `python flair-1_amd/build.py`.")
        l = C.CDLL(LIB_PATH)
        for name, (res, args) in PROTOTYPES.items():
            fn = getattr(l, name)
            fn.restype = res
            fn.argtypes = args
        _lib = l
    return _lib


def check(rc: int, what: str = ""):
    if rc != 0:
        msg = lib().flair_strerror(rc).decode()
        raise FlairHipError(f"{what}: {msg} (code {rc})" if what else f"{msg} (code {rc})")


def ptr(t):
    if t is None:
        return None
    if not t.is_cuda:
        raise FlairHipError("flair_amd kernels need tensors on a HIP device (no CPU fallback)")
    if not t.is_contiguous():
        raise FlairHipError("flair_amd kernels need contiguous tensors")
    return t.data_ptr()


def stream():
    return torch.cuda.current_stream().cuda_stream


DT_F32, DT_BF16 = 0, 1


def torch_dtype(dt: int):
    return torch.float32 if dt == DT_F32 else torch.bfloat16


def dtype_code(name) -> int:
    if name in (0, "f32", "fp32", "float32", torch.float32):
        return DT_F32
    if name in (1, "bf16", "bfloat16", torch.bfloat16):
        return DT_BF16
    raise ValueError(f"unsupported compute dtype {name!r} (use 'f32' or 'bf16')")
```

flair-1_amd/flair_amd/ops.py:

```python
from __future__ import annotations

import torch

from . import _lib as L


def _ws(nbytes, device):
    return torch.empty(int(nbytes) + 256, dtype=torch.uint8, device=device)


def _dt(t):
    return L.dtype_code(t.dtype)


def nchw_to_nhwc(x: torch.Tensor, dtype, cpad=None) -> torch.Tensor:
    N, C, H, W = x.shape
    dt = L.dtype_code(dtype)
    cpad = cpad or ((C + 7) // 8 * 8)
    y = torch.empty(N, H, W, cpad, dtype=L.torch_dtype(dt), device=x.device)
    L.check(L.lib().flair_nchw_to_nhwc(dt, L.ptr(x.float().contiguous()), L.ptr(y), N, C, H, W, cpad, L.stream()), "nchw_to_nhwc")
    return y


def nhwc_to_nchw(x: torch.Tensor, C=None) -> torch.Tensor:
# ... 18 lines not shown
    yn = torch.empty(N, Cout, Ho, Wo, dtype=torch.float32, device=x0.device) if (want_nchw or y is None) else None
    st = torch.empty(2, Cout, dtype=torch.float32, device=x0.device) if want_stats else None
    L.check(l.flair_conv2d_forward(dt, L.ptr(x0), L.ptr(x1), N, H, W, C0, C1, int(up0), L.ptr(w), L.ptr(bias), Cout, R,
                                   stride, pad, L.ptr(y), L.ptr(yn), L.ptr(st), L.ptr(ws), ws.numel(), L.stream()),
            "conv2d_forward")
    return y, yn, st


def conv2d_backward(x, w, dy, stride=1, pad=1, need_dx=True, need_dw=True):
    N, H, W, Cin = x.shape
    Cout, _, R, _ = w.shape
    dt = _dt(x)
    l = L.lib()
    ws = _ws(l.flair_conv2d_workspace_bytes(dt, N, H, W, Cin, 0, 0, Cout, R, stride, pad), x.device)
    dx = torch.empty_like(x) if need_dx else None
    dw = torch.empty_like(w) if need_dw else None
    L.check(l.flair_conv2d_backward(dt, L.ptr(x), N, H, W, Cin, L.ptr(w), Cout, R, stride, pad, L.ptr(dy), L.ptr(dx),
                                    L.ptr(dw), L.ptr(ws), ws.numel(), L.stream()), "conv2d_backward")
    return dx, dw


def _conv_ex_args(x0, w, mode=0, bias=None, stride=1, pad=1, x1=None, up0=False, want_nhwc=True, want_nchw=False, want_stats=False,
                  in_scale=None, in_shift=None, oscale=None, oshift=None, ores=None, orelu=False, out=None, accumulate=False,
                  acc_src=None, pool_c0=0, out_skip=None, skip_accumulate=False, want_preds=False, want_maxprob=False, ogelu=False,
                  bnr_y=None, bnr_out=None, bnr_scale=None, bnr_shift=None, bnr_partial=None, bnr_mask=False):
    N, H, W, C0 = x0.shape
    C1 = x1.shape[3] if x1 is not None else 0
    R = w.shape[2]
    Cout = w.shape[1] if mode else w.shape[0]
    assert (w.shape[0] if mode else w.shape[1]) == C0 + C1
    dt = _dt(x0)
    Hin, Win = (2 * H, 2 * W) if up0 else (H, W)
    p_eff = R - 1 - pad if mode == 1 else pad
    Ho, Wo = (Hin + 2 * p_eff - R) // stride + 1, (Win + 2 * p_eff - R) // stride + 1
    dev = x0.device
    if mode == 2:
        assert out is not None, "mode 2 writes into the caller's dx"
        Ho, Wo = H, W
    if out is None and want_nhwc:
        assert not accumulate or acc_src is not None, "accumulate needs the tensor to add to"
        out = (torch.empty(N, Ho // 2, Wo // 2, pool_c0, dtype=x0.dtype, device=dev) if pool_c0 else
               torch.empty(N, Ho, Wo, Cout, dtype=x0.dtype, device=dev))
    if pool_c0 and pool_c0 < Cout and out_skip is None:
        assert not skip_accumulate
        out_skip = torch.empty(N, Ho, Wo, Cout - pool_c0, dtype=x0.dtype, device=dev)
    yn = torch.empty(N, Cout, Ho, Wo, dtype=torch.float32, device=dev) if want_nchw else None
    st = torch.empty(2, Cout, dtype=torch.float32, device=dev) if want_stats else None
    pr = torch.empty(N, Ho, Wo, dtype=torch.uint8, device=dev) if want_preds else None
    mp = torch.empty(N, Ho, Wo, dtype=torch.float32, device=dev) if want_maxprob else None
    a = L.ConvEx(dtype=dt, mode=mode, x0=L.ptr(x0), x1=L.ptr(x1), N=N, H=H, W=W, C0=C0, C1=C1, up0=int(up0), w_oihw=L.ptr(w),
                 bias=L.ptr(bias), Cout=Cout, R=R, stride=stride, pad=pad, y_nhwc=L.ptr(out),
                 out_ld=out.shape[3] if out is not None else 0, y_nchw=L.ptr(yn), stats=L.ptr(st), in_scale=L.ptr(in_scale),
                 in_shift=L.ptr(in_shift), oscale=L.ptr(oscale), oshift=L.ptr(oshift), ores=L.ptr(ores), orelu=int(orelu),
                 accumulate=int(accumulate), acc_src=L.ptr(acc_src), pool_c0=pool_c0, out_skip=L.ptr(out_skip),
                 out_skip_ld=out_skip.shape[3] if out_skip is not None else 0, skip_accumulate=int(skip_accumulate),
                 preds_u8=L.ptr(pr), maxprob_f32=L.ptr(mp), ogelu=int(ogelu),
                 bnr_y=L.ptr(bnr_y), bnr_out=L.ptr(bnr_out), bnr_scale=L.ptr(bnr_scale), bnr_shift=L.ptr(bnr_shift),
                 bnr_partial=L.ptr(bnr_partial), bnr_rows=bnr_partial.shape[2] if bnr_partial is not None else 0, bnr_mask=int(bnr_mask))
    return a, {"y": out, "out_skip": out_skip, "y_nchw": yn, "stats": st, "preds": pr, "maxprob": mp}


def conv2d_ex(x0, w, **kw):
    import ctypes as C
    a, outs = _conv_ex_args(x0, w, **kw)
    l = L.lib()
    ws = _ws(l.flair_conv2d_ex_workspace_bytes(C.addressof(a)), x0.device)
    L.check(l.flair_conv2d_ex(C.addressof(a), L.ptr(ws), ws.numel(), L.stream()), "conv2d_ex")
    return outs


def conv2d_ex_grid_rows(x0, w, **kw):
    import ctypes as C
    a, _ = _conv_ex_args(x0, w, **kw)
    rows = L.lib().flair_conv2d_ex_grid_rows(C.addressof(a))
    L.check(min(rows, 0), "conv2d_ex_grid_rows")
    return rows


def conv2d_wgrad_ex(x0, dy, Cout, R=3, stride=1, pad=1, x1=None, up0=False, in_scale=None, in_shift=None, dw=None, accumulate=False,
                    want_dbias=False, cus=0, cin_real=0, fuse_y=None, fuse_coef=None, fuse_msc=None, fuse_msh=None):
    import ctypes as C
    N, H, W, C0 = x0.shape
    C1 = x1.shape[3] if x1 is not None else 0
    dt = _dt(x0)
    dev = x0.device
    if dw is None:
        assert not accumulate
        dw = torch.empty(Cout, cin_real or (C0 + C1), R, R, dtype=torch.float32, device=dev)
    db = torch.empty(Cout, dtype=torch.float32, device=dev) if want_dbias else None
    a = L.WgradEx(dtype=dt, x0=L.ptr(x0), x1=L.ptr(x1), N=N, H=H, W=W, C0=C0, C1=C1, up0=int(up0), dy=L.ptr(dy), dy_ld=dy.shape[3],
                  Cout=Cout, R=R, stride=stride, pad=pad, dw=L.ptr(dw), Cin_real=cin_real, accumulate=int(accumulate),
                  in_scale=L.ptr(in_scale), in_shift=L.ptr(in_shift), dbias=L.ptr(db), cus=cus,
                  fuse_y=L.ptr(fuse_y), fuse_coef=L.ptr(fuse_coef), fuse_msc=L.ptr(fuse_msc), fuse_msh=L.ptr(fuse_msh))
    l = L.lib()
    ws = _ws(l.flair_conv2d_wgrad_ex_workspace_bytes(C.addressof(a)), dev)
    L.check(l.flair_conv2d_wgrad_ex(C.addressof(a), L.ptr(ws), ws.numel(), L.stream()), "conv2d_wgrad_ex")
    return dw, db


def bn_relu_forward(y, gamma, beta, running_mean, running_var, training=True, residual=None, relu=True):
    C = y.shape[-1]
    rows = y.numel() // C
    out = torch.empty_like(y)
    mean = torch.empty(C, dtype=torch.float32, device=y.device)
    invstd = torch.empty(C, dtype=torch.float32, device=y.device)
    ws = _ws(L.lib().flair_bn_workspace_bytes(rows, C), y.device)
    L.check(L.lib().flair_bn_relu_forward(_dt(y), L.ptr(y), rows, C, L.ptr(gamma), L.ptr(beta), L.ptr(running_mean),
                                          L.ptr(running_var), int(training), L.ptr(residual), int(relu), L.ptr(out),
                                          L.ptr(mean), L.ptr(invstd), L.ptr(ws), ws.numel(), L.stream()), "bn_relu_forward")
    return out, mean, invstd


def bn_relu_backward(dout, out, y, gamma, mean, invstd, relu=True, want_dres=False):
    C = y.shape[-1]
    rows = y.numel() // C
    dy = torch.empty_like(y)
    dres = torch.empty_like(y) if want_dres else None
    dgamma = torch.empty(C, dtype=torch.float32, device=y.device)
    dbeta = torch.empty(C, dtype=torch.float32, device=y.device)
    ws = _ws(L.lib().flair_bn_workspace_bytes(rows, C), y.device)
    L.check(L.lib().flair_bn_relu_backward(_dt(y), L.ptr(dout), L.ptr(out), L.ptr(y), rows, C, L.ptr(gamma), L.ptr(mean),
                                           L.ptr(invstd), int(relu), L.ptr(dy), L.ptr(dres), L.ptr(dgamma), L.ptr(dbeta),
                                           L.ptr(ws), ws.numel(), L.stream()), "bn_relu_backward")
    return dy, dres, dgamma, dbeta


def bn_backward_ex(dout, y, mean, invstd, gamma=None, out=None, mscale=None, mshift=None, partial=None, pre_nblk=0, premasked=False,
                   dgamma=None, dbeta=None, accumulate_param=False, want_dy=True, dy=None, dres=None, want_dres=False,
                   dres_accumulate=False, coef=None, rc=False):
    import ctypes as C
    Cc = y.shape[-1]
    rows = y.numel() // Cc
    dev = y.device
    if dy is None and want_dy:
        dy = torch.empty_like(y)
    if dres is None and want_dres:
        assert not dres_accumulate
        dres = torch.empty_like(y)
    if dgamma is None:
        assert not accumulate_param
        dgamma = torch.empty(Cc, dtype=torch.float32, device=dev)
        dbeta = torch.empty(Cc, dtype=torch.float32, device=dev)
    if coef is None:
        coef = torch.empty(3, Cc, dtype=torch.float32, device=dev)
    a = L.BnBwdEx(dtype=_dt(y), dout=L.ptr(dout), out=L.ptr(out), y=L.ptr(y), mean=L.ptr(mean), invstd=L.ptr(invstd), gamma=L.ptr(gamma),
                  rows=rows, C=Cc, partial=L.ptr(partial), pre_nblk=pre_nblk, premasked=int(premasked), mscale=L.ptr(mscale),
                  mshift=L.ptr(mshift), dgamma=L.ptr(dgamma), dbeta=L.ptr(dbeta), accumulate_param=int(accumulate_param), dy=L.ptr(dy),
                  dres=L.ptr(dres), dres_accumulate=int(dres_accumulate), coef=L.ptr(coef))
    ws = _ws(L.lib().flair_bn_workspace_bytes(rows, Cc), dev)
    r = L.lib().flair_bn_backward_ex(C.addressof(a), L.ptr(ws), ws.numel(), L.stream())
    return _ret(r, "bn_backward_ex", {"dy": dy, "dres": dres, "dgamma": dgamma, "dbeta": dbeta, "coef": coef}, rc)


def maxpool_backward_ex(dy, idx, H, W, dx=None, accumulate=False, bnr_y=None, bnr_msc=None, bnr_msh=None, bnr_partial=None, rc=False):
    N, _, _, Cc = dy.shape
    if dx is None:
        assert not accumulate
        dx = torch.empty(N, H, W, Cc, dtype=dy.dtype, device=dy.device)
    r = L.lib().flair_maxpool_backward_ex(_dt(dy), L.ptr(dy), L.ptr(idx), L.ptr(dx), int(accumulate), N, H, W, Cc, L.ptr(bnr_y),
                                          L.ptr(bnr_msc), L.ptr(bnr_msh), L.ptr(bnr_partial), L.stream())
    return _ret(r, "maxpool_backward_ex", dx, rc)


def bn_act_maxpool(y, scale, shift, rc=False):
    N, H, W, Cc = y.shape
    act = torch.empty_like(y)
    out = torch.empty(N, H // 2, W // 2, Cc, dtype=y.dtype, device=y.device)
    idx = torch.empty(N, H // 2, W // 2, Cc, dtype=torch.uint8, device=y.device)
    r = L.lib().flair_bn_act_maxpool(_dt(y), L.ptr(y), L.ptr(scale), L.ptr(shift), L.ptr(act), L.ptr(out), L.ptr(idx), N, H, W, Cc,
                                     L.stream())
    return _ret(r, "bn_act_maxpool", (act, out, idx), rc)


def bn_act(y, scale, shift, relu=True, rc=False):
    Cc = y.shape[-1]
    out = torch.empty_like(y)
    r = L.lib().flair_bn_act(_dt(y), L.ptr(y), L.ptr(scale), L.ptr(shift), L.ptr(out), y.numel() // Cc, Cc, int(relu), L.stream())
    return _ret(r, "bn_act", out, rc)


def upcat_bwd(dcat, C0, dx0=None, dx0_accumulate=False, dskip=None, dskip_accumulate=False, rc=False):
    N, H, W, Ct = dcat.shape
    C1 = Ct - C0
    if dx0 is None:
        assert not dx0_accumulate
        dx0 = torch.empty(N, H // 2, W // 2, C0, dtype=dcat.dtype, device=dcat.device)
    if dskip is None and C1:
        assert not dskip_accumulate
        dskip = torch.empty(N, H, W, C1, dtype=dcat.dtype, device=dcat.device)
    r = L.lib().flair_upcat_bwd(_dt(dcat), L.ptr(dcat), L.ptr(dx0), int(dx0_accumulate), L.ptr(dskip), int(dskip_accumulate), N, H, W,
                                C0, C1, L.stream())
    return _ret(r, "upcat_bwd", (dx0, dskip), rc)


def ew_add_(dst, src, n=None, rc=False):
    n = dst.numel() if n is None else n
    return _ret(L.lib().flair_ew_add(_dt(dst), L.ptr(dst), L.ptr(src), n, L.stream()), "ew_add", dst, rc)


def colsum(x, C, rc=False):
    rows, ld = x.shape
    out = torch.empty(C, dtype=torch.float32, device=x.device)
    ws = _ws(L.lib().flair_bn_workspace_bytes(rows, ld), x.device)
    r = L.lib().flair_colsum(_dt(x), L.ptr(x), rows, ld, C, L.ptr(out), L.ptr(ws), ws.numel(), L.stream())
    return _ret(r, "colsum", out, rc)


def pack_weights(dtype, params, descs, arena, rc=False):
    import ctypes as C
    arr = (L.PackDesc * len(descs))(*[L.PackDesc(**d) for d in descs])
    r = L.lib().flair_pack_weights(L.dtype_code(dtype), L.ptr(params), C.addressof(arr), len(descs), L.ptr(arena), L.stream())
    return _ret(r, "pack_weights", arena, rc)


def pack_weight(dtype, w, dst, Cout, Cin, R, S, Cin_p, rows_pad, Kpad, tf, rc=False):
    r = L.lib().flair_pack_weight(L.dtype_code(dtype), L.ptr(w), L.ptr(dst), Cout, Cin, R, S, Cin_p, rows_pad, Kpad, int(tf), L.stream())
    return _ret(r, "pack_weight", dst, rc)


def maxpool_forward(x):
    N, H, W, C = x.shape
    y = torch.empty(N, H // 2, W // 2, C, dtype=x.dtype, device=x.device)
    idx = torch.empty(N, H // 2, W // 2, C, dtype=torch.uint8, device=x.device)
    L.check(L.lib().flair_maxpool_forward(_dt(x), L.ptr(x), L.ptr(y), L.ptr(idx), N, H, W, C, L.stream()), "maxpool_forward")
    return y, idx


def maxpool_backward(dy, idx, H, W):
    N, _, _, C = dy.shape
    dx = torch.empty(N, H, W, C, dtype=dy.dtype, device=dy.device)
    L.check(L.lib().flair_maxpool_backward(_dt(dy), L.ptr(dy), L.ptr(idx), L.ptr(dx), N, H, W, C, L.stream()), "maxpool_backward")
    return dx


_LABEL_KIND = {torch.uint8: 0, torch.int32: 1, torch.int64: 2}


def ce_head(logits, labels, weight=None, want_dlogits=True, want_preds="u8", confmat=None, want_targets=False,
            dlogits_nhwc=None, dlogits_ld=0):
    B, Cc, H, W = logits.shape
    kind = 3 if labels.dtype == torch.float32 else _LABEL_KIND[labels.dtype]
    dev = logits.device
    loss = torch.empty((), dtype=torch.float32, device=dev)
    dl = torch.empty_like(logits) if want_dlogits else None
    pu8 = torch.empty(B, H, W, dtype=torch.uint8, device=dev) if want_preds == "u8" else None
    pi64 = torch.empty(B, H, W, dtype=torch.int64, device=dev) if want_preds == "i64" else None
    tg = torch.empty(B, H, W, dtype=torch.int32, device=dev) if want_targets else None
    l = L.lib()
    ws = _ws(l.flair_ce_workspace_bytes(B, H, W), dev)
    L.check(l.flair_ce_head(L.ptr(logits), L.ptr(labels), kind, L.ptr(weight), B, Cc, H, W, L.ptr(loss), L.ptr(dl),
                            L.ptr(dlogits_nhwc), _dt(dlogits_nhwc) if dlogits_nhwc is not None else 0, dlogits_ld,
                            L.ptr(pu8), L.ptr(pi64), L.ptr(tg), L.ptr(confmat), L.ptr(ws), L.stream()), "ce_head")
    return loss, dl, (pu8 if pu8 is not None else pi64), tg


def softmax_argmax(logits, want="i64", want_maxprob=False):
    B, Cc, H, W = logits.shape
    dev = logits.device
    pu8 = torch.empty(B, H, W, dtype=torch.uint8, device=dev) if want == "u8" else None
    pi64 = torch.empty(B, H, W, dtype=torch.int64, device=dev) if want == "i64" else None
    mp = torch.empty(B, H, W, dtype=torch.float32, device=dev) if want_maxprob else None
    L.check(L.lib().flair_softmax_argmax(L.ptr(logits), B, Cc, H, W, L.ptr(pu8), L.ptr(pi64), L.ptr(mp), L.stream()), "softmax_argmax")
    p = pu8 if pu8 is not None else pi64
    return (p, mp) if want_maxprob else p


def confmat_update(confmat, target, pred):
    Cc = confmat.shape[0]
    L.check(L.lib().flair_confmat_update(L.ptr(target), _LABEL_KIND[target.dtype], L.ptr(pred), _LABEL_KIND[pred.dtype],
                                         target.numel(), Cc, L.ptr(confmat), L.stream()), "confmat_update")
    return confmat


def jaccard(confmat):
    Cc = confmat.shape[0]
    dev = confmat.device
    per = torch.empty(Cc, dtype=torch.float32, device=dev)
    w = torch.empty((), dtype=torch.float32, device=dev)
    m = torch.empty((), dtype=torch.float32, device=dev)
    L.check(L.lib().flair_jaccard(L.ptr(confmat), Cc, L.ptr(per), L.ptr(w), L.ptr(m), L.stream()), "jaccard")
    return per, w, m


def tiff_lzw_slot_bytes(rows_per_strip, W):
    return int(L.lib().flair_tiff_lzw_slot_bytes(int(rows_per_strip), int(W)))


def tiff_lzw_encode(u8, rows_per_strip=None):
    if u8.dtype != torch.uint8 or u8.dim() != 3:
        raise L.FlairHipError("tiff_lzw_encode needs a (B, H, W) uint8 tensor")
    B, H, W = u8.shape
    R = max(1, 8192 // W) if rows_per_strip is None else int(rows_per_strip)
    if R < 1:
        raise ValueError(f"rows_per_strip must be at least 1, got {rows_per_strip!r}")
    nstrips = -(-H // R)
    slot = tiff_lzw_slot_bytes(R, W)
    src = L.ptr(u8)
    out = torch.empty(B, nstrips, slot, dtype=torch.uint8, device=u8.device)
    counts = torch.empty(B, nstrips, dtype=torch.int32, device=u8.device)
    L.check(L.lib().flair_tiff_lzw_encode(src, B, H, W, R, L.ptr(out), slot, L.ptr(counts), L.stream()), "tiff_lzw_encode")
    return out, counts, slot, R


TIFF_INTERLEAVE = {"band": 0, "pixel": 1}


# ... 324 lines not shown
```

include/flair_hip.h:

```cpp
#ifndef FLAIR_HIP_H
#define FLAIR_HIP_H
#include <stddef.h>
#include <stdint.h>

#ifdef __cplusplus
extern "C" {
#endif

#define FLAIR_DT_F32 0
#define FLAIR_DT_BF16 1

const char* flair_strerror(int code);
int flair_version(void);

typedef struct flair_unet flair_unet_t;
int flair_unet_create(flair_unet_t** out, int in_channels, int classes, int dtype);
void flair_unet_destroy(flair_unet_t* h);
int64_t flair_unet_param_count(const flair_unet_t* h);
int64_t flair_unet_buffer_count(const flair_unet_t* h);
int flair_unet_num_tensors(const flair_unet_t* h);
int flair_unet_tensor_info(const flair_unet_t* h, int i, char* name, int name_cap, int64_t shape[4], int* ndim,
                           int64_t* offset, int* kind, int* stage);
int flair_unet_stage_range(const flair_unet_t* h, int stage, int64_t* begin, int64_t* end);
int64_t flair_unet_workspace_bytes(flair_unet_t* h, int B, int H, int W, int training);
// ... 33 lines not shown

size_t flair_ce_workspace_bytes(int B, int H, int W);
int flair_ce_head(const float* logits_nchw, const void* labels, int label_kind, const float* class_weight, int B, int C,
                  int H, int W, float* loss, float* dlogits_nchw, void* dlogits_nhwc, int dlogits_dtype, int dlogits_ld,
                  uint8_t* preds_u8, int64_t* preds_i64, int32_t* targets_i32, int64_t* confmat, void* workspace,
                  void* stream);
const void* flair_unet_logits_nhwc(const flair_unet_t* h);
int flair_ce_head_nhwc(const void* logits_nhwc, int dtype, int ld, const void* labels, int label_kind,
                       const float* class_weight, int B, int C, int H, int W, float* loss, void* dlogits_nhwc,
                       uint8_t* preds_u8, int32_t* targets_i32, int64_t* confmat, void* workspace, void* stream);
int flair_softmax_argmax_nhwc(const void* logits_nhwc, int dtype, int ld, int B, int C, int H, int W, uint8_t* preds_u8,
                              int64_t* preds_i64, float* maxprob, void* stream);
int flair_softmax_argmax(const float* logits_nchw, int B, int C, int H, int W, uint8_t* preds_u8, int64_t* preds_i64,
                         float* maxprob, void* stream);
int flair_confmat_update(const void* target, int target_kind, const void* pred, int pred_kind, int64_t n, int C,
                         int64_t* confmat, void* stream);
int flair_confmat_masks(const uint8_t* truth_raw, const uint8_t* pred, int64_t n, int C, int truth_offset, int64_t* confmat,
                        void* stream);
int flair_jaccard(const int64_t* confmat, int C, float* per_class, float* weighted, float* macro, void* stream);

int flair_feed_tiles(const uint8_t* img_u8, const uint8_t* msk_raw, const uint8_t* d4_flags, int B, int bands, int H, int W,
                     const int* channels, int n_channels, int norm_type, const double* means, const double* stds,
                     int num_classes, float* img_out, uint8_t* labels_out, void* stream);
int flair_feed_tiles_ptrs(const uint64_t* img_ptrs, const uint64_t* msk_ptrs, const uint8_t* d4_flags, int B, int bands, int H, int W,
                          const int* channels, int n_channels, int norm_type, const double* means, const double* stds,
                          int num_classes, float* img_out, uint8_t* labels_out, void* stream);
int flair_detect_convert(const float* logits_nchw, int B, int C, int S, int margin, int output_type, void* out, void* stream);
int flair_gather_tiles(const uint8_t* raster_u8, int bands, int raster_h, int raster_w, const int32_t* tiles, int B, int S,
                       const int* channels, int n_channels, int norm_type, const double* means, const double* stds,
                       float* img_out, void* stream);
int flair_detect_stitch_preds(const uint8_t* preds_u8, const float* maxprob_f32, int B, int S, int margin, const int32_t* tiles,
                              float* raster_out, int raster_h, int raster_w, void* stream);
int flair_detect_stitch(const float* logits_nchw, int B, int C, int S, int margin, int output_type, const int32_t* tiles,
                        void* raster_out, int raster_h, int raster_w, void* stream);
int flair_detect_blend_accum(const float* logits_nchw, int B, int C, int S, int margin, const int32_t* tiles, const float* cheb_weights,
                             int x_lo, int x_hi, int y_lo, int y_hi, float* ring, int raster_h, int raster_w, void* stream);
int flair_detect_blend_flush(float* ring, int C, int ring_cols, int x_lo, int x_hi, float* raster_out, int raster_h, int raster_w,
                             void* stream);
int flair_detect_stitch_max(const float* logits_nchw, int B, int C, int S, int margin, const int32_t* tiles, int x_lo, int x_hi,
                            int y_lo, int y_hi, float* raster_out, int raster_h, int raster_w, void* stream);
int flair_detect_stitch_max_preds(const uint8_t* preds_u8, const float* maxprob_f32, int B, int S, int margin, const int32_t* tiles,
                                  int x_lo, int x_hi, int y_lo, int y_hi, float* raster_out, int raster_h, int raster_w, void* stream);
int flair_detect_convert_q4(const float* logits_nchw, int B, int C, int S, int margin, int output_type, void* out, void* stream);
int flair_detect_stitch_q4(const float* logits_nchw, int B, int C, int S, int margin, int output_type, const int32_t* tiles,
                           void* raster_out, int raster_h, int raster_w, void* stream);
int flair_detect_blend_accum_q4(const float* logits_nchw, int B, int C, int S, int margin, const int32_t* tiles, const float* cheb_weights,
                                int x_lo, int x_hi, int y_lo, int y_hi, float* ring, int raster_h, int raster_w, void* stream);
int flair_detect_stitch_max_q4(const float* logits_nchw, int B, int C, int S, int margin, const int32_t* tiles, int x_lo, int x_hi,
                               int y_lo, int y_hi, float* raster_out, int raster_h, int raster_w, void* stream);

int flair_zone_window_confmat_preds(const uint8_t* preds_u8, int B, int C, int S, int margin, const int32_t* tiles,
                                    const uint8_t* truth_u8, int raster_h, int raster_w, int64_t* confmats, void* stream);
int flair_zone_window_confmat_logits(const float* logits_nchw, int B, int C, int S, int margin, const int32_t* tiles,
                                     const uint8_t* truth_u8, int raster_h, int raster_w, int64_t* confmats, void* stream);
int flair_zone_window_confmat_logits_q4(const float* logits_nchw, int B, int C, int S, int margin, const int32_t* tiles,
                                        const uint8_t* truth_u8, int raster_h, int raster_w, int64_t* confmats, void* stream);
int flair_zone_window_confmat_raster(const float* raster, int B, int C, int S, int margin, const int32_t* tiles, const uint8_t* truth_u8,
                                     int raster_h, int raster_w, int64_t* confmats, void* stream);
int flair_zone_raster_confmat(const float* raster, const uint8_t* truth_u8, int raster_h, int raster_w, int C, int64_t* confmat,
                              void* stream);
int flair_zone_error_map(const float* raster, const uint8_t* truth_u8, int raster_h, int raster_w, int K, const int32_t* row_origins,
                         int n_rows, const int32_t* col_origins, int n_cols, double sigma, int radius, uint8_t* mask_ws,
                         int32_t* colsum_ws, int32_t* counts_ws, double* tmp_ws, double* error_map, void* stream);

long flair_tiff_lzw_slot_bytes(int rows_per_strip, int W);
int flair_tiff_lzw_encode(const uint8_t* img, int B, int H, int W, int rows_per_strip, uint8_t* out, long slot_bytes, int32_t* counts,
                          void* stream);
long flair_tiff_lzw_tile_slot_bytes(int tile, int samples);
int flair_tiff_lzw_encode_tiles(const void* raster, int src_f32, const float* scale, int bands, int H, int W, int tile, int interleave,
                                long first_stream, long n_streams, uint8_t* out, long slot_bytes, int32_t* counts, void* stream);
int flair_tiff_pack_streams(const uint8_t* slots, long slot_bytes, const int32_t* counts, const int64_t* dst_off, long n_streams, uint8_t* dst,
                            long dst_bytes, void* stream);
int flair_tiff_lzw_decode_max_strip(void);
int flair_tiff_lzw_decode(const uint8_t* src, long src_bytes, const int64_t* strip_src_off, const int32_t* strip_src_len,
                          const int64_t* strip_dst_off, const int32_t* strip_dst_len, const int32_t* strip_mode, long nstrips, uint8_t* dst,
                          long dst_bytes, int32_t* status, void* stream);
int flair_tiff_lzw_decode_chunks_cap(void);
int flair_tiff_lzw_decode_chunks_window(void);
int flair_tiff_lzw_decode_chunks(const uint8_t* src, long src_bytes, const int64_t* src_off, const int32_t* src_len, const int32_t* dst_len,
                                 const int32_t* mode, long nchunks, uint8_t* scratch, long slot_bytes, int32_t* status, void* stream);
int flair_tiff_chunks_to_planes(const uint8_t* scratch, long slot_bytes, const int32_t* chunks, const int32_t* status, long nchunks,
                                int max_rows, int samples, int predictor, uint8_t* planes, int bands, int H, int W, void* stream);
int flair_tiff_chunks_to_batch(const uint8_t* scratch, long slot_bytes, const int32_t* chunks, const int32_t* status, long nchunks,
                               int max_rows, uint8_t* planes, int n_planes, int H, int W, void* stream);

int flair_sgd_step(float* params, const float* grads, int64_t n, float lr, void* stream);
int flair_add_rowvec_nchw(float* x, const float* v, int N, int C, int H, int W, void* stream);
int flair_add_rowvec_nhwc(int dtype, void* x, const float* v, int N, int H, int W, int C, void* stream);
int flair_add_rowvec_nhwc_to(int dtype, const void* x, const float* v, void* y, int N, int H, int W, int C, void* stream);
int flair_rowvec_grad_nhwc(int dtype, const void* dx, float* dv, int N, int H, int W, int C, void* stream);

size_t flair_conv2d_workspace_bytes(int dtype, int N, int H, int W, int C0, int C1, int up0, int Cout, int R,
                                    int stride, int pad);
int flair_conv2d_forward(int dtype, const void* x0, const void* x1, int N, int H, int W, int C0, int C1, int up0,
                         const float* w_oihw, const float* bias, int Cout, int R, int stride, int pad, void* y_nhwc,
                         float* y_nchw, float* stats, void* workspace, size_t workspace_bytes, void* stream);
int flair_conv2d_backward(int dtype, const void* x0, int N, int H, int W, int Cin, const float* w_oihw, int Cout, int R,
                          int stride, int pad, const void* dy_nhwc, void* dx_nhwc, float* dw_oihw, void* workspace,
                          size_t workspace_bytes, void* stream);
typedef struct flair_conv_ex {
  int dtype, mode;
  const void* x0; const void* x1;
  int N, H, W, C0, C1, up0;
  const float* w_oihw; const float* bias;
  int Cout, R, stride, pad;
  void* y_nhwc; int out_ld;
  float* y_nchw; float* stats;
  const float* in_scale; const float* in_shift;
  const float* oscale; const float* oshift; const void* ores; int orelu;
  int accumulate; const void* acc_src;
  int pool_c0; void* out_skip; int out_skip_ld; int skip_accumulate;
  uint8_t* preds_u8; float* maxprob_f32;
  int ogelu;
  const void* bnr_y; const void* bnr_out; const float* bnr_scale; const float* bnr_shift;
  float* bnr_partial; int bnr_rows; int bnr_mask;
} flair_conv_ex_t;
typedef struct flair_wgrad_ex {
  int dtype;
  const void* x0; const void* x1;
  int N, H, W, C0, C1, up0;
  const void* dy; int dy_ld;
  int Cout, R, stride, pad;
  float* dw; int Cin_real; int accumulate;
  const float* in_scale; const float* in_shift;
  float* dbias; int cus;
  const void* fuse_y; const float* fuse_coef; const float* fuse_msc; const float* fuse_msh;
} flair_wgrad_ex_t;
size_t flair_conv2d_ex_workspace_bytes(const flair_conv_ex_t* p);
int flair_conv2d_ex(const flair_conv_ex_t* p, void* workspace, size_t workspace_bytes, void* stream);
int flair_conv2d_ex_grid_rows(const flair_conv_ex_t* p);
size_t flair_conv2d_wgrad_ex_workspace_bytes(const flair_wgrad_ex_t* p);
int flair_conv2d_wgrad_ex(const flair_wgrad_ex_t* p, void* workspace, size_t workspace_bytes, void* stream);
size_t flair_bn_workspace_bytes(int64_t rows, int C);
int flair_bn_relu_forward(int dtype, const void* y, int64_t rows, int C, const float* gamma, const float* beta,
                          float* running_mean, float* running_var, int training, const void* residual, int relu,
                          void* out, float* save_mean, float* save_invstd, void* workspace, size_t workspace_bytes,
                          void* stream);
int flair_bn_relu_backward(int dtype, const void* dout, const void* out, const void* y, int64_t rows, int C,
                           const float* gamma, const float* save_mean, const float* save_invstd, int relu, void* dy,
                           void* dres, float* dgamma, float* dbeta, void* workspace, size_t workspace_bytes,
                           void* stream);
typedef struct flair_bn_bwd_ex {
  int dtype;
  const void* dout; const void* out; const void* y;
  const float* mean; const float* invstd; const float* gamma;
  int64_t rows; int C;
  float* partial; int pre_nblk; int premasked;
  const float* mscale; const float* mshift;
  float* dgamma; float* dbeta; int accumulate_param;
  void* dy; void* dres; int dres_accumulate;
  float* coef;
} flair_bn_bwd_ex_t;
int flair_bn_backward_ex(const flair_bn_bwd_ex_t* p, void* workspace, size_t workspace_bytes, void* stream);
int flair_maxpool_forward(int dtype, const void* x, void* y, uint8_t* idx, int N, int H, int W, int C, void* stream);
int flair_maxpool_backward(int dtype, const void* dy, const uint8_t* idx, void* dx, int N, int H, int W, int C,
                           void* stream);
int flair_maxpool_backward_ex(int dtype, const void* dy, const uint8_t* idx, void* dx, int accumulate, int N, int H, int W, int C,
                              const void* bnr_y, const float* bnr_msc, const float* bnr_msh, float* bnr_partial, void* stream);
int flair_bn_act(int dtype, const void* y, const float* scale, const float* shift, void* out, int64_t rows, int C, int relu,
                 void* stream);
int flair_bn_act_maxpool(int dtype, const void* y, const float* scale, const float* shift, void* act, void* out, uint8_t* idx, int N,
                         int H, int W, int C, void* stream);
int flair_upcat_bwd(int dtype, const void* dcat, void* dx0, int dx0_accumulate, void* dskip, int dskip_accumulate, int N, int H, int W,
                    int C0, int C1, void* stream);
int flair_ew_add(int dtype, void* dst, const void* src, int64_t n, void* stream);
int flair_colsum(int dtype, const void* x, int64_t rows, int ld, int C, float* out, void* workspace, size_t workspace_bytes,
                 void* stream);
typedef struct flair_pack_desc {
  int64_t w_off; uint64_t dst_off;
  int Cout, Cin, R, S, Cin_p, rows_pad, Kpad, tf;
  int r0, rstep, Rc, s0, sstep, Sc;
} flair_pack_desc_t;
int flair_pack_weights(int dtype, const float* params, const flair_pack_desc_t* descs, int n, void* base, void* stream);
int flair_pack_weight(int dtype, const float* w_oihw, void* dst, int Cout, int Cin, int R, int S, int Cin_p, int rows_pad, int Kpad,
                      int tf, void* stream);
int flair_nchw_to_nhwc(int dtype, const float* x_nchw, void* y_nhwc, int N, int C, int H, int W, int Cpad, void* stream);
int flair_nhwc_to_nchw(int dtype, const void* x_nhwc, float* y_nchw, int N, int C, int H, int W, int Cpad, void* stream);

int flair_sf_layernorm(int dtype, const void* x, const float* gamma, const float* beta, void* y, int64_t rows, int C, float eps,
                       void* stream);
int flair_sf_dwconv3x3_gelu(int dtype, const void* x, const float* w, const float* bias, void* y, int B, int H, int W, int C,
                            void* stream);
int flair_sf_bilinear_nhwc(int dtype, const void* x, void* y, int B, int h, int w, int C, int H, int W, int ld, void* stream);
int flair_sf_bilinear_nchw_f32(const float* x, float* y, int64_t planes, int h, int w, int H, int W, void* stream);
int flair_sf_slice_cols(int dtype, const float* src, int ld, int col0, int ncols, int64_t rows, void* dst, void* stream);
int flair_sf_fuse_bias(const float* wf, int D, const float* b3, const float* b2, const float* b1, const float* b0,
                       const float* scale, const float* shift, float* shift2, void* stream);
int flair_sf_upsample_sum_bn_relu(int dtype, const void* g0, const void* g1, const void* g2, const void* g3, const float* scale,
                                  const float* shift2, void* z, int B, int H, int W, int D, void* stream);
int flair_sf_ffn_fused_ok(int dtype, int C, int H, int W);
int flair_sf_ffn_dw_pack(const float* w, const float* b, float* out, int nch, void* stream);
int flair_sf_ffn_fused(const void* x, const float* ln_g, const float* ln_b, const void* w1, const float* b1, const float* dwp,
                       const void* w2, const float* b2, void* out, int B, int H, int W, int C, float eps, const float* ln2_g,
                       const float* ln2_b, void* out_ln, void* stream);
int flair_sf_head_fused_ok(int dtype, int H, int W, int C0, int D, int labels);
int flair_sf_head_wint(void* wint_bf16_128x96, void* stream);
int flair_sf_head_fused(const void* f0, const void* w0, const void* g1, const void* g2, const void* g3, const void* wint,
                        const float* scale, const float* shift2, const void* wc, const float* bc, float* out, int B, int H, int W,
                        int D, int labels, void* stream);
int flair_sf_attention(int dtype, const void* q, const void* k, const void* v, void* out, int B, int N, int Nk, int hidden,
                       int kv_ld, void* stream);
int flair_swin_window_attention(int dtype, const void* qkv, const float* qkv_bias, const float* table, void* out, int B, int H,
                                int W, int C, int heads, int shift, void* stream);
int flair_swin_layernorm(int dtype, const void* x, const float* gamma, const float* beta, void* y, int64_t rows, int C, int ld,
                         float eps, void* stream);
int flair_swin_patch_merge_ln(int dtype, const void* x, const float* gamma, const float* beta, void* y, int B, int H, int W, int C,
                              float eps, void* stream);
int flair_swin_adaptive_avgpool(int dtype, const void* x, int ld, void* y, int B, int h, int w, int C, int S, void* stream);
int flair_swin_bilinear_add(int dtype, const void* x, void* y, int B, int h, int w, int C, int H, int W, void* stream);

int flair_metadata_mlp_forward(const float* x, const float* const w[3], const float* const b[3], const float* const mask[3],
                               float* h1, float* h2, float* out, int B, void* stream);
int flair_metadata_mlp_backward(const float* x, const float* h1, const float* h2, const float* out, const float* const w[3],
                                const float* const mask[3], const float* dout, int B, float* const dw[3], float* const db[3],
                                float* scratch, void* stream);

int flair_profile_start(int max_records);
int flair_profile_stop(void);
int flair_profile_kernel(int i, char* name, int name_cap, double* total_ms, int64_t* launches, double* flops,
                         double* bytes);

typedef struct flair_segformer flair_segformer_t;
int flair_segformer_create(flair_segformer_t** out, int in_channels, int num_labels, const int depths[4],
                           const int hidden_sizes[4], const int num_heads[4], const int sr_ratios[4],
                           int decoder_hidden_size, int dtype);
void flair_segformer_destroy(flair_segformer_t* h);
int64_t flair_segformer_param_count(const flair_segformer_t* h);
int flair_segformer_num_tensors(const flair_segformer_t* h);
int flair_segformer_tensor_info(const flair_segformer_t* h, int i, char* name, int name_cap, int64_t shape[4], int* ndim,
                                int64_t* offset, int* kind);
int64_t flair_segformer_workspace_bytes(flair_segformer_t* h, int B, int H, int W);
void flair_segformer_weights_changed(flair_segformer_t* h);
int flair_segformer_forward(flair_segformer_t* h, const float* params, const float* x_nchw, float* logits_quarter_nchw,
                            float* logits_full_nchw, int B, int H, int W, void* workspace, size_t workspace_bytes,
                            void* stream);

typedef struct flair_upernet flair_upernet_t;
int flair_upernet_create(flair_upernet_t** out, int in_channels, int num_labels, int embed_dim, const int depths[4],
                         const int num_heads[4], int window_size, int hidden_size, const int pool_scales[4],
                         int auxiliary_in_channels, int auxiliary_channels, int dtype);
void flair_upernet_destroy(flair_upernet_t* h);
int64_t flair_upernet_param_count(const flair_upernet_t* h);
int flair_upernet_num_tensors(const flair_upernet_t* h);
int flair_upernet_tensor_info(const flair_upernet_t* h, int i, char* name, int name_cap, int64_t shape[4], int* ndim,
                              int64_t* offset, int* kind);
int64_t flair_upernet_workspace_bytes(flair_upernet_t* h, int B, int H, int W);
void flair_upernet_weights_changed(flair_upernet_t* h);
int flair_upernet_forward(flair_upernet_t* h, const float* params, const float* x_nchw, float* logits_nchw, int B, int H, int W,
                          void* workspace, size_t workspace_bytes, void* stream);
int flair_upernet_forward_quarter(flair_upernet_t* h, const float* params, const float* x_nchw, float* logits_quarter_nchw, int B, int H,
                                  int W, void* workspace, size_t workspace_bytes, void* stream);

int flair_tune_set(const char* key, int value);
int flair_debug_buffer(void* device_u64);

#ifdef __cplusplus
}
#endif
#endif
```

Before: 2831 tiles/s.

## Fuse 16-channel 3x3 dgrad and wgrad into one halo-tiled backward kernel

Adds a fused backward kernel for 16-channel stride-1 3x3 convolutions at full resolution. One pass stages the gradient halo and the BN-ReLU-applied input, then computes dgrad (with BN-reduce statistics) and wgrad slabs from the same LDS tiles. By default it is enabled for decoder unit convs (mode 3), which removes separate dgrad/wgrad launches and repeated reads of large 512x512x16 activations. The cost is a more complex kernel with double-buffered register prefetch and an extra slab reduction. A standalone C API and a step-planning workspace path are also added.

```diff
diff --git a/flair-1_amd/build.py b/flair-1_amd/build.py
--- a/flair-1_amd/build.py
+++ b/flair-1_amd/build.py
@@ -9,7 +9,7 @@
 OUT_DIR = os.path.join(HERE, "flair_amd")
 OBJ_DIR = os.path.join(HERE, "build")
 LIB = os.path.join(OUT_DIR, "libflair_hip.so")
-SOURCES = ["conv_igemm.hip", "conv_halo.hip", "conv_hg.hip", "wgrad.hip", "wgrad_halo.hip", "wgrad_hg.hip", "stem.hip", "batchnorm.hip", "misc.hip", "ce_head.hip", "feed.hip", "zone_stitch.hip", "zone_metrics.hip", "tiff_lzw.hip", "tiff_read.hip", "unet.hip", "capi.hip", "prof.hip", "tune.hip", "metadata_mlp.hip", "tf_exec.hip", "segformer_ops.hip", "segformer.hip", "swin_ops.hip", "upernet.hip"]
+SOURCES = ["conv_igemm.hip", "conv_halo.hip", "conv_hg.hip", "wgrad.hip", "wgrad_halo.hip", "bwd_halo16.hip", "wgrad_hg.hip", "stem.hip", "batchnorm.hip", "misc.hip", "ce_head.hip", "feed.hip", "zone_stitch.hip", "zone_metrics.hip", "tiff_lzw.hip", "tiff_read.hip", "unet.hip", "capi.hip", "prof.hip", "tune.hip", "metadata_mlp.hip", "tf_exec.hip", "segformer_ops.hip", "segformer.hip", "swin_ops.hip", "upernet.hip"]
 FLAGS = ["--offload-arch=gfx950", "-O3", "-std=c++17", "-fPIC", "-Wall", "-Wno-unused-function"]
 SOURCE_FLAGS = {src: ["-fno-slp-vectorize"] for src in ("feed.hip", "zone_stitch.hip", "zone_metrics.hip")}
 if os.environ.get("FLAIR_STAMPS") == "1":
diff --git a/flair-1_amd/csrc/bwd_halo16.h b/flair-1_amd/csrc/bwd_halo16.h
--- /dev/null
+++ b/flair-1_amd/csrc/bwd_halo16.h
@@ -0,0 +1,38 @@
+#pragma once
+#include "common.h"
+
+namespace flair {
+
+struct Bwd16Args {
+  const void* g;
+  const void* gy;
+  const float* gcoef;
+  const float* gmsc;
+  const float* gmsh;
+  const void* x;
+  const float* in_scale;
+  const float* in_shift;
+  const void* w;
+  int Kpad;
+  void* dx;
+  const float* bnr_scale;
+  const float* bnr_shift;
+  float* bnr_partial;
+  int bnr_C, bnr_cols;
+  float* slabs;
+  float* dw;
+  int Cout, Cin_real;
+  float* dbias;
+  float* dbias_partial;
+  int N, H, W;
+  int grid;
+};
+
+constexpr int FLAIR_BWD16_FUSE_DEFAULT = 3;
+enum { BWD16_HEAD = 0, BWD16_UNIT = 1 };
+bool bwd16_fusable(int dtype, int flavour, const ConvArgs& a, const WgradArgs& w);
+int bwd16_grid(const WgradArgs& w);
+size_t bwd16_workspace_bytes(int grid);
+int launch_bwd16(const Bwd16Args& a, hipStream_t s);
+
+}
diff --git a/flair-1_amd/csrc/bwd_halo16.hip b/flair-1_amd/csrc/bwd_halo16.hip
--- /dev/null
+++ b/flair-1_amd/csrc/bwd_halo16.hip
@@ -0,0 +1,319 @@
+#include "bwd_halo16.h"
+
+#include <string.h>
+
+#include "halo_stage.h"
+#include "launch.h"
+#include "mma.h"
+#include "ops.h"
+#include "tile_direct.h"
+#include "tile_store.h"
+#include "tr_frag.h"
+#include "tune.h"
+
+namespace flair {
+
+void launch_wgrad_reduce(const float* partial, float* dw, int splits, int Cout, int Cout_pad, int Kpad, int Cin,
+                         int Cin_real, int R, int S, int accumulate, hipStream_t s);
+
+namespace {
+
+typedef bf16_t T;
+constexpr int TH = 8, TW = 32, HW_ = TW + 2, HPIX = (TH + 2) * HW_;
+constexpr int C = 16, CH = 8, CPP = C / CH;
+constexpr int HIT = (HPIX * CPP + 255) / 256;
+constexpr int KF = 4 * CH, KW = (9 * C + KF - 1) / KF * KF, NK = KW / KF;
+constexpr int WROW = KW * (int)sizeof(T) + 16;
+constexpr int PSTR = C * (int)sizeof(T) + 16;
+constexpr int KG = 9 * C;
+constexpr int WOFF = 0, GOFF = (C * WROW + 255) / 256 * 256, XOFF = GOFF + (HPIX * PSTR + 255) / 256 * 256,
+              YOFF = XOFF + (HPIX * PSTR + 255) / 256 * 256,
+              SOFF = YOFF + TH * TW * C * (int)sizeof(T), COFF = SOFF + 4 * C * 2 * 4, SMEM = COFF + 9 * C * 4;
+static_assert(HPIX * PSTR >= 9 * 4 * 64 * 4 && HPIX * PSTR >= 256 * CH * 4, "merge and bias buffers reuse the images");
+
+template <bool UNIT>
+__global__ __launch_bounds__(256, 2) void bwd16_fused_kernel(const Bwd16Args a, int ntiles) {
+  extern __shared__ __attribute__((aligned(16))) unsigned char smem[];
+  unsigned char* wl = smem + WOFF;
+  unsigned char* gimg = smem + GOFF;
+  unsigned char* ximg = smem + XOFF;
+  unsigned char* yraw = smem + YOFF;
+  float* st = reinterpret_cast<float*>(smem + SOFF);
+  float* ctab = reinterpret_cast<float*>(smem + COFF);
+  const int t = threadIdx.x, lane = t & 63, wave = t >> 6;
+  const int lr = lane & 15, lq = lane >> 4;
+  const int H = a.H, W = a.W;
+  const int tiles_x = W / TW, tiles_y = H / TH;
+  const int G = gridDim.x;
+  const HaloSrc<T> gsrc{(const T*)a.g, H, W, C, 0, 0};
+  const HaloSrc<T> ysrc{(const T*)a.gy, H, W, C, 0, 0};
+  const HaloSrc<T> xsrc{(const T*)a.x, H, W, C, 0, 0};
+  T* __restrict__ dx = (T*)a.dx;
+
+  {
+    const T* __restrict__ wp = (const T*)a.w;
+    for (int it = t; it < C * (KW - 9 * C) / CH; it += 256) {
+      const int row = it / ((KW - 9 * C) / CH), pc = it - row * ((KW - 9 * C) / CH);
+      *reinterpret_cast<u32x4*>(wl + row * WROW + (9 * C + pc * CH) * (int)sizeof(T)) = u32x4{0u, 0u, 0u, 0u};
+    }
+    for (int it = t; it < C * 9 * CPP; it += 256) {
+      const int row = it / (9 * CPP), rem = it - row * (9 * CPP);
+      const int tap = rem / CPP, ch = rem - tap * CPP;
+      *reinterpret_cast<u32x4*>(wl + row * WROW + rem * 16) = *reinterpret_cast<const u32x4*>(wp + (long)row * a.Kpad + tap * C + ch * CH);
+    }
+  }
+  if constexpr (UNIT) {
+    if (t < 5 * C) ctab[t] = t < 3 * C ? a.gcoef[t] : (t < 4 * C ? a.gmsc[t - 3 * C] : a.gmsh[t - 4 * C]);
+  }
+  if (t >= 5 * C && t < 9 * C) {
+    const int j = (t - 5 * C) / C, c = t % C;
+    ctab[t] = j == 0 ? a.in_scale[c] : j == 1 ? a.in_shift[c] : j == 2 ? a.bnr_scale[c] : a.bnr_shift[c];
+  }
+  float r1[4], r2[4];
+#pragma unroll
+  for (int e = 0; e < 4; ++e) { r1[e] = 0.f; r2[e] = 0.f; }
+  const bool bnr_per_tile = a.bnr_cols != G;
+  f32x4_t wacc[9];
+#pragma unroll
+  for (int tp = 0; tp < 9; ++tp) wacc[tp] = f32x4_t{0.f, 0.f, 0.f, 0.f};
+  float bsum[CH];
+#pragma unroll
+  for (int e = 0; e < CH; ++e) bsum[e] = 0.f;
+
+  u32x4 gA[HIT], yA[HIT], xA[HIT], gB[HIT], yB[HIT], xB[HIT];
+  unsigned bitsA = 0, bitsB = 0;
+  auto tile_load = [&](int tile, u32x4 (&gr)[HIT], u32x4 (&yr)[HIT], u32x4 (&xr)[HIT], unsigned& bits) {
+    const bool tok = tile < ntiles;
+    int n, y0, x0;
+    tile_decode<TW, TH>(tok ? tile : 0, tiles_x, tiles_y, n, y0, x0);
+    halo_gather<T, TW, TH, CPP, 256>(gsrc, tok, n, y0, x0, H, W, t, gr, bits);
+    if constexpr (UNIT) halo_gather<T, TW, TH, CPP, 256>(ysrc, tok, n, y0, x0, H, W, t, yr, bits);
+    halo_gather<T, TW, TH, CPP, 256>(xsrc, tok, n, y0, x0, H, W, t, xr, bits);
+  };
+  auto tile_stage = [&](const u32x4 (&gr)[HIT], const u32x4 (&yr)[HIT], const u32x4 (&xr)[HIT], unsigned bits) {
+#pragma unroll
+    for (int k = 0; k < HIT; ++k) {
+      const int it = t + 256 * k;
+      if (it < HPIX * CPP) {
+        const int hp = it / CPP, ch = it - hp * CPP;
+        const unsigned mask = 0u - ((bits >> k) & 1u);
+        u32x4 gv = gr[k];
+        if constexpr (UNIT) {
+          float d[CH], yy[CH], gg[CH];
+          chunk_to_f<T>(__builtin_bit_cast(uint4, gr[k]), d);
+          chunk_to_f<T>(__builtin_bit_cast(uint4, yr[k]), yy);
+          const float* cf = ctab + ch * CH;
+#pragma unroll
+          for (int e = 0; e < CH; ++e) {
+            d[e] = fmaf(yy[e], cf[3 * C + e], cf[4 * C + e]) > 0.f ? d[e] : 0.f;
+            gg[e] = fmaf(cf[e], d[e], fmaf(cf[C + e], yy[e], cf[2 * C + e]));
+          }
+          gv = __builtin_bit_cast(u32x4, f_to_chunk<T>(gg));
+        }
+        *reinterpret_cast<u32x4*>(gimg + hp * PSTR + ch * 16) = gv & mask;
+        *reinterpret_cast<u32x4*>(ximg + hp * PSTR + ch * 16) = chunk_bn_relu<T>(xr[k], ctab + 5 * C + ch * CH, ctab + 6 * C + ch * CH) & mask;
+        const int hy = hp / HW_, hx = hp - hy * HW_;
+        if (hy >= 1 && hy <= TH && hx >= 1 && hx <= TW)
+          *reinterpret_cast<u32x4*>(yraw + ((hy - 1) * TW + hx - 1) * (C * (int)sizeof(T)) + ch * 16) = xr[k];
+      }
+    }
+  };
+
+  tile_load(blockIdx.x, gA, yA, xA, bitsA);
+  tile_load(blockIdx.x + G, gB, yB, xB, bitsB);
+  __syncthreads();
+  tile_stage(gA, yA, xA, bitsA);
+  __syncthreads();
+  auto do_tile = [&](int tile, u32x4 (&ldg)[HIT], u32x4 (&ldy)[HIT], u32x4 (&ldx)[HIT], unsigned& ldbits, const u32x4 (&stg)[HIT],
+                     const u32x4 (&sty)[HIT], const u32x4 (&stx)[HIT], const unsigned& stbits) {
+    tile_load(tile + 2 * G, ldg, ldy, ldx, ldbits);
+    __builtin_amdgcn_sched_barrier(0);
+    f32x4_t acc[4];
+#pragma unroll
+    for (int i = 0; i < 4; ++i) acc[i] = f32x4_t{0.f, 0.f, 0.f, 0.f};
+    auto rdk = [&](u32x4 (&af)[4], u32x4& bfr, int j) {
+      const int k0 = j * KF + lq * CH;
+      int tap = k0 / C;
+      const int c = k0 - tap * C;
+      tap = tap > 8 ? 8 : tap;
+      const int r = tap / 3, s = tap - 3 * r;
+#pragma unroll
+      for (int i = 0; i < 4; ++i) {
+        const int py = 2 * wave + (i >> 1), px = (i & 1) * 16 + lr;
+        af[i] = *reinterpret_cast<const u32x4*>(gimg + ((py + r) * HW_ + px + s) * PSTR + c * (int)sizeof(T));
+      }
+      bfr = *reinterpret_cast<const u32x4*>(wl + direct_row_channel<1>(0, lr) * WROW + k0 * (int)sizeof(T));
+    };
+    auto mmk = [&](const u32x4 (&af)[4], const u32x4& bfr) {
+#pragma unroll
+      for (int i = 0; i < 4; ++i) Mma<T>::run(bfr, af[i], acc[i]);
+    };
+#pragma unroll
+    for (int j = 0; j < NK; ++j) {
+      u32x4 af[4], bfr;
+      rdk(af, bfr, j);
+      mmk(af, bfr);
+    }
+    {
+      int n, y0, x0;
+      tile_decode<TW, TH>(tile, tiles_x, tiles_y, n, y0, x0);
+#pragma unroll
+      for (int i = 0; i < 4; ++i) {
+        const int py = 2 * wave + (i >> 1), px = (i & 1) * 16 + lr;
+        float f[4], yv[4];
+#pragma unroll
+        for (int rr = 0; rr < 4; ++rr) f[rr] = Elem<T>::to_f(Elem<T>::from_f(acc[i][rr]));
+        LaneVec<T, 4>::store(dx + ((long)(n * H + y0 + py) * W + x0 + px) * C + 4 * lq, f);
+        LaneVec<T, 4>::load(reinterpret_cast<const T*>(yraw + (py * TW + px) * (C * (int)sizeof(T))) + 4 * lq, yv);
+#pragma unroll
+        for (int e = 0; e < 4; ++e) {
+          const float d = Elem<T>::to_f(Elem<T>::from_f(f[e]));
+          const float dm = fmaf(yv[e], ctab[7 * C + 4 * lq + e], ctab[8 * C + 4 * lq + e]) > 0.f ? d : 0.f;
+          r1[e] += dm;
+          r2[e] = fmaf(dm, yv[e], r2[e]);
+        }
+      }
+    }
+#pragma unroll
+    for (int yy = 0; yy < 2; ++yy) {
+      const int y = wave * 2 + yy;
+      const u32x4 af = HFrag<T>::template load<PSTR>(gimg, (y + 1) * HW_ + 1, 0, lane);
+#pragma unroll
+      for (int tp = 0; tp < 9; ++tp) {
+        const int r = tp / 3, s = tp - 3 * r;
+        const u32x4 bf = HFrag<T>::template load<PSTR>(ximg, (y + r) * HW_ + s, 0, lane);
+        Mma<T>::run(af, bf, wacc[tp]);
+      }
+    }
+    if constexpr (!UNIT) {
+      if (a.dbias_partial) {
+#pragma unroll
+        for (int k = 0; k < 2; ++k) {
+          const int px = (t + 256 * k) / CPP, py = px / TW, pxx = px - py * TW;
+          float f[CH];
+          chunk_to_f<T>(*reinterpret_cast<const uint4*>(gimg + ((py + 1) * HW_ + pxx + 1) * PSTR + (t % CPP) * 16), f);
+#pragma unroll
+          for (int e = 0; e < CH; ++e) bsum[e] += f[e];
+        }
+      }
+    }
+    if (bnr_per_tile) {
+      direct_stats_wave<1>(r1, r2, st, C, 0, wave, lane);
+      __syncthreads();
+      tile_stats_write<4, C>(st, a.bnr_partial, a.bnr_C, 0, a.bnr_cols, tile, t);
+#pragma unroll
+      for (int e = 0; e < 4; ++e) { r1[e] = 0.f; r2[e] = 0.f; }
+    }
+    __syncthreads();
+    tile_stage(stg, sty, stx, stbits);
+    __syncthreads();
+  };
+  for (int tile = blockIdx.x; tile < ntiles; tile += 2 * G) {
+    do_tile(tile, gA, yA, xA, bitsA, gB, yB, xB, bitsB);
+    if (tile + G < ntiles) do_tile(tile + G, gB, yB, xB, bitsB, gA, yA, xA, bitsA);
+  }
+
+  if (!bnr_per_tile) {
+    direct_stats_wave<1>(r1, r2, st, C, 0, wave, lane);
+    __syncthreads();
+    tile_stats_write<4, C>(st, a.bnr_partial, a.bnr_C, 0, G, blockIdx.x, t);
+  }
+  if constexpr (!UNIT) {
+    if (a.dbias_partial) {
+      float* bs = reinterpret_cast<float*>(ximg);
+#pragma unroll
+      for (int e = 0; e < CH; ++e) bs[t * CH + e] = bsum[e];
+      __syncthreads();
+      if (t < C) {
+        const int chunk = t / CH, e = t - chunk * CH;
+        float x = 0.f;
+        for (int th = chunk; th < 256; th += CPP) x += bs[th * CH + e];
+        a.dbias_partial[(long)t * G + blockIdx.x] = x;
+      }
+    }
+  }
+  float* red = reinterpret_cast<float*>(gimg);
+  for (int w = 1; w < 4; ++w) {
+    if (wave == w) {
+#pragma unroll
+      for (int tp = 0; tp < 9; ++tp)
+#pragma unroll
+        for (int e = 0; e < 4; ++e) red[(tp * 4 + e) * 64 + lane] = wacc[tp][e];
+    }
+    __syncthreads();
+    if (wave == 0) {
+#pragma unroll
+      for (int tp = 0; tp < 9; ++tp)
+#pragma unroll
+        for (int e = 0; e < 4; ++e) wacc[tp][e] += red[(tp * 4 + e) * 64 + lane];
+    }
+    __syncthreads();
+  }
+  if (wave == 0) {
+    float* __restrict__ part = a.slabs + (long)blockIdx.x * C * KG;
+#pragma unroll
+    for (int tp = 0; tp < 9; ++tp)
+#pragma unroll
+      for (int e = 0; e < 4; ++e) part[(long)(lq * 4 + e) * KG + tp * C + lr] = wacc[tp][e];
+  }
+}
+
+}
+
+bool bwd16_fusable(int dtype, int flavour, const ConvArgs& a, const WgradArgs& w) {
+  const int mode = tune("FLAIR_BWD16_FUSE", FLAIR_BWD16_FUSE_DEFAULT);
+  if (!(mode == 1 || (mode == 2 && flavour == BWD16_HEAD) || (mode == 3 && flavour == BWD16_UNIT))) return false;
+  if (dtype != DT_BF16) return false;
+  if (a.R != 3 || a.S != 3 || a.out_mul != 1 || a.in_div != 1 || a.pad != 1) return false;
+  if (a.C0 != C || a.C1 || a.up0 || a.Cout != C || a.out_ld != C || !a.out) return false;
+  if (a.Hout != a.Hin || a.Wout != a.Win || (a.Hout % TH) || (a.Wout % TW)) return false;
+  if (a.accumulate || a.acc_src || a.pool_c0 || a.out_skip || a.in_scale || a.stats || a.oscale || a.oshift || a.bias || a.ores ||
+      a.orelu || a.out_nchw || a.out_sub || a.ncls || a.preds_u8 || a.ce_lab8 || a.ogelu)
+    return false;
+  if (!a.bnr_partial || !a.bnr_y || a.bnr_out || a.bnr_mask || a.bnr_C != C) return false;
+  if (w.R != 3 || w.S != 3 || w.stride != 1 || w.pad != 1 || w.C0 != C || w.C1 || w.up0 || w.dy_ld != C || w.Cout > C || w.accumulate)
+    return false;
+  if (w.N != a.N || w.Hin != a.Hout || w.Win != a.Wout || w.dy != a.src0 || w.fuse_y) return false;
+  if (!w.in_scale || !w.in_shift || w.x0 != a.bnr_y) return false;
+  return true;
+}
+
+int bwd16_grid(const WgradArgs& w) {
+  const long ntiles = (long)w.N * w.Hin * w.Win / (TH * TW);
+  long wgs = tune("FLAIR_BWD16_WGS", 0);
+  if (wgs <= 0) wgs = (long)(wgrad_halo_workspace_bytes(DT_BF16, w) / ((size_t)C * KG * sizeof(float)));
+  if (wgs < 1) wgs = 1;
+  return (int)(wgs < ntiles ? wgs : ntiles);
+}
+
+size_t bwd16_workspace_bytes(int grid) { return (size_t)grid * C * KG * sizeof(float); }
+
+int launch_bwd16(const Bwd16Args& a, hipStream_t s) {
+  if ((a.H % TH) || (a.W % TW) || a.bnr_C != C || a.Cout > C) return -2;
+  const long ntiles = (long)a.N * a.H * a.W / (TH * TW);
+  const bool unit = a.gy != nullptr;
+  const int grid = a.grid;
+  if (grid < 1 || grid > ntiles) return -2;
+  if (a.bnr_cols != grid && a.bnr_cols != ntiles) return -6;
+  if (a.dbias && (unit || !a.dbias_partial || grid > WGRAD_DBIAS_ROWS)) return -6;
+  Bwd16Args k = a;
+  if (!a.dbias) k.dbias_partial = nullptr;
+  ConvArgs ca;
+  memset(&ca, 0, sizeof(ca));
+  ca.N = a.N; ca.Hout = a.H; ca.Wout = a.W; ca.C0 = C; ca.Cout = C; ca.Kg = KG;
+  struct { int N, H, W, Cout, C0, C1, up0, dy_ld; } wa = {a.N, a.H, a.W, a.Cout, C, 0, 0, C};
+  const ProfCost cd = conv_prof_cost(ca, sizeof(T), false, false), cw = wgrad3x3_prof_cost(wa, sizeof(T));
+  const ProfCost cost{cd.flops + cw.flops, cd.bytes + (double)ntiles * TH * TW * C * sizeof(T) * (unit ? 2 : 1)};
+  const int rc = unit ? launch_kernel<bwd16_fused_kernel<true>>("bwd16_fused_unit_bf16", cost, dim3(grid), dim3(256), SMEM, s, k, (int)ntiles)
+                      : launch_kernel<bwd16_fused_kernel<false>>("bwd16_fused_head_bf16", cost, dim3(grid), dim3(256), SMEM, s, k, (int)ntiles);
+  if (rc) return rc;
+  launch_wgrad_reduce(a.slabs, a.dw, grid, a.Cout, C, KG, C, a.Cin_real, 3, 3, 0, s);
+  if (a.dbias) {
+    const int rb = partial_rows_sum(a.dbias_partial, grid, a.Cout, a.dbias, s);
+    if (rb) return rb;
+  }
+  const hipError_t e = hipGetLastError();
+  return e == hipSuccess ? 0 : (int)e;
+}
+
+}
diff --git a/flair-1_amd/csrc/capi.hip b/flair-1_amd/csrc/capi.hip
--- a/flair-1_amd/csrc/capi.hip
+++ b/flair-1_amd/csrc/capi.hip
@@ -644,6 +644,60 @@
                      p->premasked, (hipStream_t)stream);
 }
 
+static size_t bwd16_ex_pack_bytes() { return (size_t)round_up(16L * conv_kpad(DT_BF16, 9 * 16) * 2, 256); }
+
+static void bwd16_ex_wgrad(const flair_bwd16_ex_t* p, WgradArgs& w) {
+  wgrad_args(w, ConvInput{p->x, nullptr, 16, 0, 0, p->N, p->H, p->W}, 3, 1, 1, p->g, 16, p->Cout, p->dw, 16);
+  w.in_scale = p->in_scale; w.in_shift = p->in_shift;
+}
+
+size_t flair_bwd16_ex_workspace_bytes(const flair_bwd16_ex_t* p) {
+  if (!p || p->N < 1 || p->H < 1 || p->W < 1 || (p->H % 8) || (p->W % 32)) return 0;
+  WgradArgs w;
+  bwd16_ex_wgrad(p, w);
+  return bwd16_ex_pack_bytes() + (size_t)round_up((long)bwd16_workspace_bytes(bwd16_grid(w)), 256) +
+         (size_t)round_up((long)WGRAD_DBIAS_ROWS * 16 * 4, 256) + 256;
+}
+
+int flair_bwd16_ex_grid_rows(const flair_bwd16_ex_t* p) {
+  if (!p || p->N < 1 || p->H < 1 || p->W < 1) return -1;
+  if ((p->H % 8) || (p->W % 32)) return -2;
+  WgradArgs w;
+  bwd16_ex_wgrad(p, w);
+  return bwd16_grid(w);
+}
+
+int flair_bwd16_ex(const flair_bwd16_ex_t* p, void* workspace, size_t wsb, void* stream) {
+  if (!p || !p->g || !p->x || !p->in_scale || !p->in_shift || !p->w_oihw || !p->dx || !p->bnr_scale || !p->bnr_shift || !p->bnr_partial ||
+      !p->dw || !workspace || p->N < 1 || p->H < 1 || p->W < 1)
+    return -1;
+  if (p->gy && (!p->gcoef || !p->gmsc || !p->gmsh || p->dbias)) return -1;
+  if (p->Cout < 1 || p->Cout > 16 || (p->H % 8) || (p->W % 32)) return -2;
+  hipStream_t s = (hipStream_t)stream;
+  WgradArgs w;
+  bwd16_ex_wgrad(p, w);
+  const int grid = bwd16_grid(w);
+  if (p->bnr_rows < grid) return -100;
+  OpArena ar(workspace, wsb);
+  const int Kpad = conv_kpad(DT_BF16, 9 * 16);
+  void* wp = ar.get((size_t)16 * Kpad * 2);
+  Bwd16Args f;
+  memset(&f, 0, sizeof(f));
+  f.slabs = (float*)ar.get(bwd16_workspace_bytes(grid));
+  f.grid = grid;
+  if (p->dbias) f.dbias_partial = (float*)ar.get((size_t)WGRAD_DBIAS_ROWS * 16 * 4);
+  if (ar.bad) return -100;
+  const int rc = pack_weight(DT_BF16, p->w_oihw, wp, p->Cout, 16, 3, 3, 16, 16, Kpad, 1, s);
+  if (rc) return rc;
+  f.g = p->g; f.gy = p->gy; f.gcoef = p->gcoef; f.gmsc = p->gmsc; f.gmsh = p->gmsh;
+  f.x = p->x; f.in_scale = p->in_scale; f.in_shift = p->in_shift;
+  f.w = wp; f.Kpad = Kpad; f.dx = p->dx;
+  f.bnr_scale = p->bnr_scale; f.bnr_shift = p->bnr_shift; f.bnr_partial = p->bnr_partial; f.bnr_C = 16; f.bnr_cols = grid;
+  f.dw = p->dw; f.Cout = p->Cout; f.Cin_real = 16; f.dbias = p->dbias;
+  f.N = p->N; f.H = p->H; f.W = p->W;
+  return launch_bwd16(f, s);
+}
+
 int flair_maxpool_backward_ex(int dtype, const void* dy, const uint8_t* idx, void* dx, int accumulate, int N, int H, int W, int C,
                               const void* bnr_y, const float* bnr_msc, const float* bnr_msh, float* bnr_partial, void* stream) {
   if (!dy || !idx || !dx || N < 1 || H < 1 || W < 1 || C < 1) return -1;
diff --git a/flair-1_amd/csrc/tr_frag.h b/flair-1_amd/csrc/tr_frag.h
--- /dev/null
+++ b/flair-1_amd/csrc/tr_frag.h
@@ -0,0 +1,37 @@
+#pragma once
+#include "common.h"
+
+namespace flair {
+
+template <typename T> struct HFrag;
+template <> struct HFrag<bf16_t> {
+  static constexpr int KSTEP = 32;
+  template <int STRIDE>
+  __device__ static __forceinline__ u32x4 load(const unsigned char* img, int row0, int cb, int lane) {
+    const int g = lane >> 4, i = lane & 15, q = i >> 2, p = i & 3;
+    typedef __attribute__((address_space(3))) s16x4_t* lds_p;
+    s16x4_t lo = __builtin_amdgcn_ds_read_tr16_b64_v4i16((lds_p)(img + (row0 + 8 * g + 2 * q) * STRIDE + cb + 8 * p));
+    s16x4_t hi = __builtin_amdgcn_ds_read_tr16_b64_v4i16((lds_p)(img + (row0 + 8 * g + 2 * q + 1) * STRIDE + cb + 8 * p));
+    u32x4 r;
+    r.x = (unsigned)(unsigned short)lo[0] | ((unsigned)(unsigned short)lo[1] << 16);
+    r.y = (unsigned)(unsigned short)lo[2] | ((unsigned)(unsigned short)lo[3] << 16);
+    r.z = (unsigned)(unsigned short)hi[0] | ((unsigned)(unsigned short)hi[1] << 16);
+    r.w = (unsigned)(unsigned short)hi[2] | ((unsigned)(unsigned short)hi[3] << 16);
+    return r;
+  }
+};
+template <> struct HFrag<float> {
+  static constexpr int KSTEP = 16;
+  template <int STRIDE>
+  __device__ static __forceinline__ u32x4 load(const unsigned char* img, int row0, int cb, int lane) {
+    const int g = lane >> 4, i = lane & 15;
+    u32x4 r;
+    r.x = *reinterpret_cast<const unsigned*>(img + (row0 + g) * STRIDE + cb + 4 * i);
+    r.y = *reinterpret_cast<const unsigned*>(img + (row0 + 4 + g) * STRIDE + cb + 4 * i);
+    r.z = *reinterpret_cast<const unsigned*>(img + (row0 + 8 + g) * STRIDE + cb + 4 * i);
+    r.w = *reinterpret_cast<const unsigned*>(img + (row0 + 12 + g) * STRIDE + cb + 4 * i);
+    return r;
+  }
+};
+
+}
diff --git a/flair-1_amd/csrc/unet.h b/flair-1_amd/csrc/unet.h
--- a/flair-1_amd/csrc/unet.h
+++ b/flair-1_amd/csrc/unet.h
@@ -2,6 +2,7 @@
 #include <string>
 #include <vector>
 
+#include "bwd_halo16.h"
 #include "ops.h"
 
 namespace flair {
@@ -158,6 +159,8 @@
   int sole_producer(const Act& a) const;
   int residual_producer(const Act& a) const;
   void attach_bn_reduce(ConvArgs& a, const Act& target);
+  bool bwd16_ok(int flavour, const ConvArgs& a, const WgradArgs& w, const Act& x) const;
+  void bwd16_run(Bwd16Args& f, const ConvArgs& a, const WgradArgs& w, const Act& x);
   std::vector<GradBuf> gbufs_;
   const void* acc_src_next_ = nullptr;
   bool bwd_fuse() const;
@@ -165,6 +168,7 @@
   void* grad_peek(const Act& a);
 
   size_t plan_bytes(int B, int H, int W, int training);
+  size_t plan_step_bytes(int B, int H, int W);
   void build_table();
   int add_conv(const std::string& name, int cin, int cout, int k, int stride, int pad, bool bias, int stage);
   int add_bn(const std::string& name, int c, int stage);
diff --git a/flair-1_amd/csrc/unet.hip b/flair-1_amd/csrc/unet.hip
--- a/flair-1_amd/csrc/unet.hip
+++ b/flair-1_amd/csrc/unet.hip
@@ -568,7 +568,6 @@
   const ConvDesc& c = convs[u.conv];
   const BnDesc& b = bns[u.bn];
   const long rows = u.y.rows();
-  void* dy = alloc((size_t)u.y.elems() * dtype_size(dtype));
   const int pre_nblk = u.bnr_nblk;
   const bool masked = u.bnr_masked && pre_nblk > 0;
   float* partial = pre_nblk > 0 ? u.bnr_partial : alloc_f((long)bn_bwd_blocks(rows) * 2 * b.C);
@@ -577,6 +576,10 @@
   const void* acc_src = acc_src_next_;
   acc_src_next_ = nullptr;
   const bool mask_from_y = u.relu && u.res_unit < 0 && !u.res.p;
+  const bool cand16 = dtype == DT_BF16 && need_dgrad && !dres && !upcat && !dx_override && mask_from_y && pre_nblk > 0 && !masked &&
+                      !acc_src && c.R == 3 && c.stride == 1 && c.pad == 1 && u.y.C == 16 && b.C == 16 && c.Cin_p == 16 && !u.in1.p &&
+                      !u.up0 && u.in0.lz_scale;
+  void* dy = cand16 ? const_cast<void*>(dout) : alloc((size_t)u.y.elems() * dtype_size(dtype));
   WgradArgs w;
   wgrad_args(w, conv_input(u.in0, u.in1, u.up0), c.R, c.stride, c.pad, dy, u.y.C, c.Cout, grads_ + c.w_off, c.Cin);
   const bool fuse_apply = !need_dgrad && !dres && mask_from_y && wgrad_bnapply_fusable(dtype, w);
@@ -636,13 +639,25 @@
       }
     }
   }
+  w.in_scale = u.in0.lz_scale; w.in_shift = u.in0.lz_shift;
+  const bool fuse16 = cand16 && dg == DG_PLAIN && bwd16_ok(BWD16_UNIT, a, w, u.in0);
+  if (cand16 && !fuse16) {
+    dy = alloc((size_t)u.y.elems() * dtype_size(dtype));
+    w.dy = dy; a.src0 = dy;
+  }
   const bool nomask = masked && !dres && bwd_fuse();
   RUN(bn_backward(dtype, dout, (u.relu && !mask_from_y && !nomask) ? u.out.p : nullptr, u.y.p, u.mean, u.invstd, params_ + b.g_off,
-                  rows, b.C, partial, coef, grads_ + b.g_off, grads_ + b.b_off, 0, fuse_apply ? nullptr : dy, dres,
+                  rows, b.C, partial, coef, grads_ + b.g_off, grads_ + b.b_off, 0, (fuse_apply || fuse16) ? nullptr : dy, dres,
                   dres_acc ? 1 : 0, (mask_from_y && !nomask) ? u.scale : nullptr, (mask_from_y && !nomask) ? u.shift : nullptr,
                   pre_nblk, nomask ? 1 : 0, s_));
+  if (fuse16) {
+    Bwd16Args f;
+    memset(&f, 0, sizeof(f));
+    f.g = dout; f.gy = u.y.p; f.gcoef = coef; f.gmsc = u.scale; f.gmsh = u.shift;
+    bwd16_run(f, a, w, u.in0);
+    return;
+  }
   if (fuse_apply) { w.dy = dout; w.fuse_y = u.y.p; w.fuse_coef = coef; w.fuse_msc = u.scale; w.fuse_msh = u.shift; }
-  w.in_scale = u.in0.lz_scale; w.in_shift = u.in0.lz_shift;
   w.cus = side_cus();
   w.partial = (float*)alloc(wgrad_workspace_bytes(dtype, w));
   {
@@ -660,24 +675,45 @@
   }
 }
 
+bool UNet::bwd16_ok(int flavour, const ConvArgs& a, const WgradArgs& w, const Act& x) const {
+  if (!bwd16_fusable(dtype, flavour, a, w)) return false;
+  if (tune("FLAIR_BWD16_WGS", 0) > 0) return true;
+  const int p = sole_producer(x);
+  if (p < 0) return false;
+  const int nblk = units_[p].bnr_nblk, grid = bwd16_grid(w);
+  if (nblk == grid || nblk == (long)a.N * a.Hout * a.Wout / 256) return true;
+  static bool told = false;
+  if (!told && !dry_) {
+    told = true;
+    fprintf(stderr, "flair: fused 16-channel backward not used: the data gradient's %d partial columns are not the weight gradient's grid "
+                    "of %d workgroups (FLAIR_BWD16_WGS overrides)\n", nblk, grid);
+  }
+  return false;
+}
+
+void UNet::bwd16_run(Bwd16Args& f, const ConvArgs& a, const WgradArgs& w, const Act& x) {
+  const int p = sole_producer(x);
+  if (p < 0) { if (!err_) err_ = -6; return; }
+  Unit& up = units_[p];
+  const int grid = bwd16_grid(w);
+  const long ntiles = (long)a.N * a.Hout * a.Wout / 256;
+  if (up.bnr_nblk != grid && up.bnr_nblk != ntiles) { up.bnr_partial = alloc_f((long)grid * 2 * up.y.C); up.bnr_nblk = grid; }
+  f.x = x.p; f.in_scale = w.in_scale; f.in_shift = w.in_shift;
+  f.w = a.w; f.Kpad = a.Kpad; f.dx = a.out;
+  f.bnr_scale = a.bnr_scale; f.bnr_shift = a.bnr_shift; f.bnr_partial = up.bnr_partial; f.bnr_C = a.bnr_C; f.bnr_cols = up.bnr_nblk;
+  f.slabs = (float*)alloc(bwd16_workspace_bytes(grid));
+  f.grid = grid;
+  f.dw = w.dw; f.Cout = w.Cout; f.Cin_real = w.Cin_real;
+  f.N = a.N; f.H = a.Hout; f.W = a.Wout;
+  RUN(launch_bwd16(f, s_));
+}
+
 void UNet::head_bwd_impl(const void* dl) {
   const ConvDesc& c = convs.back();
   Act none;
   WgradArgs w;
   wgrad_args(w, conv_input(dec_out_, none, false), c.R, c.stride, c.pad, dl, c.Cout_p, c.Cout, grads_ + c.w_off, c.Cin);
   w.in_scale = dec_out_.lz_scale; w.in_shift = dec_out_.lz_shift;
-  w.partial = (float*)alloc(wgrad_workspace_bytes(dtype, w));
-  const bool fuse_db = wgrad_dbias_fusable(dtype, w);
-  if (fuse_db) { w.dbias = grads_ + c.b_off; w.dbias_partial = alloc_f((long)WGRAD_DBIAS_ROWS * c.Cout_p); }
-  {
-    hipStream_t ws = wgrad_stream();
-    RUN(launch_wgrad(dtype, w, ws));
-  }
-  if (!fuse_db) {
-    const long rows = dec_out_.rows();
-    float* partial = alloc_f((long)bn_bwd_blocks(rows) * c.Cout_p);
-    RUN(colsum(dtype, dl, rows, c.Cout_p, c.Cout, partial, grads_ + c.b_off, s_));
-  }
   ConvArgs a;
   conv_dgrad_args(a, dtype, ConvInput{dl, nullptr, c.Cout_p, 0, 0, dec_out_.N, dec_out_.H, dec_out_.W}, c.R, c.stride, c.pad, dec_out_.H,
                   dec_out_.W, c.Cin_p);
@@ -686,7 +722,25 @@
   a.out = grad_of(dec_out_, &acc);
   a.out_ld = c.Cin_p; a.accumulate = acc ? 1 : 0;
   attach_bn_reduce(a, dec_out_);
-  RUN(launch_conv(dtype, a, s_));
+  const bool fuse_db = wgrad_dbias_fusable(dtype, w);
+  const bool fuse16 = bwd16_ok(BWD16_HEAD, a, w, dec_out_);
+  if (fuse_db) { w.dbias = grads_ + c.b_off; w.dbias_partial = alloc_f((long)WGRAD_DBIAS_ROWS * c.Cout_p); }
+  if (fuse16) {
+    Bwd16Args f;
+    memset(&f, 0, sizeof(f));
+    f.g = dl; f.dbias = w.dbias; f.dbias_partial = w.dbias_partial;
+    bwd16_run(f, a, w, dec_out_);
+  } else {
+    w.partial = (float*)alloc(wgrad_workspace_bytes(dtype, w));
+    hipStream_t ws = wgrad_stream();
+    RUN(launch_wgrad(dtype, w, ws));
+  }
+  if (!fuse_db) {
+    const long rows = dec_out_.rows();
+    float* partial = alloc_f((long)bn_bwd_blocks(rows) * c.Cout_p);
+    RUN(colsum(dtype, dl, rows, c.Cout_p, c.Cout, partial, grads_ + c.b_off, s_));
+  }
+  if (!fuse16) RUN(launch_conv(dtype, a, s_));
 }
 
 void UNet::decoder_bwd_impl() {
@@ -864,7 +918,30 @@
 
 size_t UNet::workspace_bytes(int B, int H, int W, int training) const {
   UNet scratch(in_channels, classes, dtype);
-  return scratch.plan_bytes(B, H, W, training);
+  return training == 2 ? scratch.plan_step_bytes(B, H, W) : scratch.plan_bytes(B, H, W, training);
+}
+
+size_t UNet::plan_step_bytes(int B, int H, int W) {
+  begin(nullptr, 0, nullptr, true);
+  fwd_common_begin(nullptr, nullptr, B, H, W, 1);
+  const int lazy_env = tune("FLAIR_LAZY_BN", 1);
+  lazy_ok_ = lazy_env != 0;
+  lazy_max_c_ = lazy_env >= 2 ? 32 : 16;
+  encoder_fwd_impl(nullptr);
+  alloc_act(f_[5].N, f_[5].H, f_[5].W, f_[5].C);
+  decoder_fwd_impl();
+  head_fwd_impl(nullptr, FwdOpts());
+  alloc((size_t)dec_out_.rows() * convs.back().Cout_p * dtype_size(dtype));
+  grads_ = nullptr;
+  head_bwd_impl(nullptr);
+  decoder_bwd_impl();
+  encoder_bwd_impl();
+  const size_t need = top_ + (1 << 20);
+  dry_ = false;
+  base_ = nullptr;
+  units_.clear();
+  gbufs_.clear();
+  return need;
 }
 
 size_t UNet::plan_bytes(int B, int H, int W, int training) {
diff --git a/flair-1_amd/csrc/wgrad_halo.hip b/flair-1_amd/csrc/wgrad_halo.hip
--- a/flair-1_amd/csrc/wgrad_halo.hip
+++ b/flair-1_amd/csrc/wgrad_halo.hip
@@ -2,6 +2,7 @@
 #include "halo_stage.h"
 #include "launch.h"
 #include "mma.h"
+#include "tr_frag.h"
 #include "tune.h"
 #include "ops.h"
 
@@ -13,37 +14,6 @@
 namespace {
 
 constexpr int TH = 8, TW = 32, HH = TH + 2, HW_ = TW + 2, HPIX = HH * HW_;
-
-template <typename T> struct HFrag;
-template <> struct HFrag<bf16_t> {
-  static constexpr int KSTEP = 32;
-  template <int STRIDE>
-  __device__ static __forceinline__ u32x4 load(const unsigned char* img, int row0, int cb, int lane) {
-    const int g = lane >> 4, i = lane & 15, q = i >> 2, p = i & 3;
-    typedef __attribute__((address_space(3))) s16x4_t* lds_p;
-    s16x4_t lo = __builtin_amdgcn_ds_read_tr16_b64_v4i16((lds_p)(img + (row0 + 8 * g + 2 * q) * STRIDE + cb + 8 * p));
-    s16x4_t hi = __builtin_amdgcn_ds_read_tr16_b64_v4i16((lds_p)(img + (row0 + 8 * g + 2 * q + 1) * STRIDE + cb + 8 * p));
-    u32x4 r;
-    r.x = (unsigned)(unsigned short)lo[0] | ((unsigned)(unsigned short)lo[1] << 16);
-    r.y = (unsigned)(unsigned short)lo[2] | ((unsigned)(unsigned short)lo[3] << 16);
-    r.z = (unsigned)(unsigned short)hi[0] | ((unsigned)(unsigned short)hi[1] << 16);
-    r.w = (unsigned)(unsigned short)hi[2] | ((unsigned)(unsigned short)hi[3] << 16);
-    return r;
-  }
-};
-template <> struct HFrag<float> {
-  static constexpr int KSTEP = 16;
-  template <int STRIDE>
-  __device__ static __forceinline__ u32x4 load(const unsigned char* img, int row0, int cb, int lane) {
-    const int g = lane >> 4, i = lane & 15;
-    u32x4 r;
-    r.x = *reinterpret_cast<const unsigned*>(img + (row0 + g) * STRIDE + cb + 4 * i);
-    r.y = *reinterpret_cast<const unsigned*>(img + (row0 + 4 + g) * STRIDE + cb + 4 * i);
-    r.z = *reinterpret_cast<const unsigned*>(img + (row0 + 8 + g) * STRIDE + cb + 4 * i);
-    r.w = *reinterpret_cast<const unsigned*>(img + (row0 + 12 + g) * STRIDE + cb + 4 * i);
-    return r;
-  }
-};
 
 struct WgHaloArgs {
   const void* x0; const void* x1; int C0, C1, up0;
diff --git a/flair-1_amd/flair_amd/_lib.py b/flair-1_amd/flair_amd/_lib.py
--- a/flair-1_amd/flair_amd/_lib.py
+++ b/flair-1_amd/flair_amd/_lib.py
@@ -68,6 +68,9 @@
     "flair_bn_relu_forward": (i32, [i32, vp, i64, i32, vp, vp, vp, vp, i32, vp, i32, vp, vp, vp, vp, sz, vp]),
     "flair_bn_relu_backward": (i32, [i32, vp, vp, vp, i64, i32, vp, vp, vp, i32, vp, vp, vp, vp, vp, sz, vp]),
     "flair_bn_backward_ex": (i32, [vp, vp, sz, vp]),
+    "flair_bwd16_ex_workspace_bytes": (sz, [vp]),
+    "flair_bwd16_ex_grid_rows": (i32, [vp]),
+    "flair_bwd16_ex": (i32, [vp, vp, sz, vp]),
     "flair_maxpool_backward_ex": (i32, [i32, vp, vp, vp, i32, i32, i32, i32, i32, vp, vp, vp, vp, vp]),
     "flair_bn_act": (i32, [i32, vp, vp, vp, vp, i64, i32, i32, vp]),
     "flair_bn_act_maxpool": (i32, [i32, vp, vp, vp, vp, vp, vp, i32, i32, i32, i32, vp]),
@@ -190,6 +193,12 @@
                 ("dy", vp), ("dres", vp), ("dres_accumulate", i32), ("coef", vp)]
 
 
+class Bwd16Ex(C.Structure):
+    _fields_ = [("g", vp), ("gy", vp), ("gcoef", vp), ("gmsc", vp), ("gmsh", vp), ("x", vp), ("in_scale", vp), ("in_shift", vp),
+                ("w_oihw", vp), ("Cout", i32), ("N", i32), ("H", i32), ("W", i32), ("dx", vp),
+                ("bnr_scale", vp), ("bnr_shift", vp), ("bnr_partial", vp), ("bnr_rows", i32), ("dw", vp), ("dbias", vp)]
+
+
 class PackDesc(C.Structure):
     _fields_ = [("w_off", i64), ("dst_off", C.c_uint64),
                 ("Cout", i32), ("Cin", i32), ("R", i32), ("S", i32), ("Cin_p", i32), ("rows_pad", i32), ("Kpad", i32), ("tf", i32),
diff --git a/flair-1_amd/flair_amd/ops.py b/flair-1_amd/flair_amd/ops.py
--- a/flair-1_amd/flair_amd/ops.py
+++ b/flair-1_amd/flair_amd/ops.py
@@ -194,6 +194,27 @@
     return _ret(r, "bn_backward_ex", {"dy": dy, "dres": dres, "dgamma": dgamma, "dbeta": dbeta, "coef": coef}, rc)
 
 
+def bwd16_ex(g, x, in_scale, in_shift, w, bnr_scale, bnr_shift, gy=None, gcoef=None, gmsc=None, gmsh=None, want_dbias=False, rc=False):
+    import ctypes as C
+    N, H, W, _ = g.shape
+    dev = g.device
+    Cout = w.shape[0]
+    a = L.Bwd16Ex(g=L.ptr(g), gy=L.ptr(gy), gcoef=L.ptr(gcoef), gmsc=L.ptr(gmsc), gmsh=L.ptr(gmsh), x=L.ptr(x), in_scale=L.ptr(in_scale),
+                  in_shift=L.ptr(in_shift), w_oihw=L.ptr(w), Cout=Cout, N=N, H=H, W=W, bnr_scale=L.ptr(bnr_scale), bnr_shift=L.ptr(bnr_shift))
+    l = L.lib()
+    rows = l.flair_bwd16_ex_grid_rows(C.addressof(a))
+    if rows < 0:
+        return _ret(rows, "bwd16_ex_grid_rows", None, rc)
+    dx = torch.full_like(g, float("nan"))
+    dw = torch.full((Cout, 16, 3, 3), float("nan"), dtype=torch.float32, device=dev)
+    db = torch.full((Cout,), float("nan"), dtype=torch.float32, device=dev) if want_dbias else None
+    part = torch.full((2, 16, rows), float("nan"), dtype=torch.float32, device=dev)
+    a.dx, a.dw, a.dbias, a.bnr_partial, a.bnr_rows = L.ptr(dx), L.ptr(dw), L.ptr(db), L.ptr(part), rows
+    ws = _ws(l.flair_bwd16_ex_workspace_bytes(C.addressof(a)), dev)
+    r = l.flair_bwd16_ex(C.addressof(a), L.ptr(ws), ws.numel(), L.stream())
+    return _ret(r, "bwd16_ex", {"dx": dx, "dw": dw, "dbias": db, "partial": part, "rows": rows}, rc)
+
+
 def maxpool_backward_ex(dy, idx, H, W, dx=None, accumulate=False, bnr_y=None, bnr_msc=None, bnr_msh=None, bnr_partial=None, rc=False):
     N, _, _, Cc = dy.shape
     if dx is None:
diff --git a/include/flair_hip.h b/include/flair_hip.h
--- a/include/flair_hip.h
+++ b/include/flair_hip.h
@@ -209,6 +209,18 @@
   float* coef;
 } flair_bn_bwd_ex_t;
 int flair_bn_backward_ex(const flair_bn_bwd_ex_t* p, void* workspace, size_t workspace_bytes, void* stream);
+typedef struct flair_bwd16_ex {
+  const void* g; const void* gy; const float* gcoef; const float* gmsc; const float* gmsh;
+  const void* x; const float* in_scale; const float* in_shift;
+  const float* w_oihw; int Cout;
+  int N, H, W;
+  void* dx;
+  const float* bnr_scale; const float* bnr_shift; float* bnr_partial; int bnr_rows;
+  float* dw; float* dbias;
+} flair_bwd16_ex_t;
+size_t flair_bwd16_ex_workspace_bytes(const flair_bwd16_ex_t* p);
+int flair_bwd16_ex_grid_rows(const flair_bwd16_ex_t* p);
+int flair_bwd16_ex(const flair_bwd16_ex_t* p, void* workspace, size_t workspace_bytes, void* stream);
 int flair_maxpool_forward(int dtype, const void* x, void* y, uint8_t* idx, int N, int H, int W, int C, void* stream);
 int flair_maxpool_backward(int dtype, const void* dy, const uint8_t* idx, void* dx, int N, int H, int W, int C,
                            void* stream);
```

New measurement: 2875 tiles/s, median of 6. +1.6%, better.
